# yex33/ReSpaSol

Measured on AMD Instinct MI355X. Metric: CSR SpMV GFLOP/s + achieved HBM GB/s (fp64 vs fp32), SuiteSparse set, 1/2/4/8 GPU, higher is better.
Workload: dtype f64; 1 GPU; big-set CSR SpMV fp64, 15 matrices per step; matrices=15, nnz_stored_total=268386865, parallelism=1 GPU, launch=rsp_spmv_batch (1 launch(es) of <= 32 matrices per step part): whole step

## Files before the change

### respasol_amd/csrc/rsp_api.cpp

```cpp

#include "rsp_internal.h"
#include "spmv_pack.h"

#include <atomic>

using namespace rsp_api;

using rsp::SpmvBlock;
using rsp::SpmvLongRow;
using rsp::SpmvTile;

namespace {
std::atomic<unsigned long long> g_plan_next{1};
unsigned long long plan_new_gen() { return g_plan_next.fetch_add(1); }
}


struct SpmvBounds {
    size_t nblocks, nlong, nslots;
};

static SpmvBounds spmv_bounds(int64_t rows, int64_t nnz, int cap) {
    SpmvBounds b;
    size_t q = (size_t)(nnz / cap) + 1;
    size_t l = (size_t)(nnz / rsp::kSpmvLongRow) + 1;
    b.nlong = q;
    b.nslots = 2 * q + 1;
    b.nblocks = 6 * q + 2 * l + (size_t)(rows / rsp::kSpmvMaxRows) + 8;
    b.nblocks += std::min<size_t>(b.nblocks, 8192);
    return b;
}

struct SpmvLayout {
    size_t off_long, off_part, off_cbase, off_poff, off_cidx, off_runs, bytes;
};
static SpmvLayout spmv_layout(const SpmvBounds &b, size_t elem, int64_t nnz, size_t run_ints = 0) {
    SpmvLayout l;
    l.off_long = align256(b.nblocks * sizeof(SpmvBlock));
    l.off_part = l.off_long + align256(b.nlong * sizeof(SpmvLongRow));
    l.off_cbase = l.off_part + align256(b.nslots * 2 * elem);
    l.off_poff = l.off_cbase + align256(b.nblocks * sizeof(int));
    l.off_cidx = l.off_poff + align256(b.nblocks * sizeof(int));
    l.off_runs = l.off_cidx + align256((size_t)std::max<int64_t>(nnz, 0) * sizeof(uint16_t));
    l.bytes = l.off_runs + align256(run_ints * sizeof(int));
    return l;
}

static int tile_cap(rsp_datatype_t t) {
    return t == RSP_R_64F ? SpmvTile<double>::kMaxNnz : SpmvTile<float>::kMaxNnz;
}
static int chunk_cap(rsp_datatype_t t) {
    return t == RSP_R_64F ? SpmvTile<double>::kChunk : SpmvTile<float>::kChunk;
}
static int spmv_row_align(rsp_handle_t h, rsp_datatype_t t) {
    const int e = (int)elem_size(t);
    return (h->spmv_variant & 64) ? 128 / e : (h->spmv_variant & 128) ? 64 / e : 1;
}

static int build_spmv_plan(const int *rp, int m, int cap, int chunk, rsp_an::hvec<SpmvBlock> &blocks,
                           rsp_an::hvec<SpmvLongRow> &longrows, int *nslots,
                           int maxrows = rsp::kSpmvMaxRows, int row_align = 1) {
    blocks.clear();
    longrows.clear();
    int slots = 0;
    int r = 0;
    while (r < m) {
        int len = rp[r + 1] - rp[r];
        if (len > rsp::kSpmvLongRow) {
            if (len <= chunk) {
                SpmvBlock b;
                b.r0 = r;
                b.r1 = rsp::kSpmvWholeRow;
                b.k0 = rp[r];
                b.k1 = rp[r + 1];
                blocks.push_back(b);
                r++;
                continue;
            }
            SpmvLongRow lr;
            lr.row = r;
            lr.first = slots;
            lr.nchunks = 0;
            lr.pad = 0;
            for (int k = rp[r]; k < rp[r + 1]; k += chunk) {
                SpmvBlock b;
                b.r0 = r;
                b.r1 = -(slots + 1);
                b.k0 = k;
                b.k1 = std::min(k + chunk, rp[r + 1]);
                blocks.push_back(b);
                slots++;
                lr.nchunks++;
            }
            longrows.push_back(lr);
            r++;
            continue;
        }
        int start = r, nnz = 0;
        while (r < m && r - start < maxrows) {
            int l = rp[r + 1] - rp[r];
            if (l > rsp::kSpmvLongRow || (r > start && nnz + l > cap)) break;
            nnz += l;
            r++;
        }
        if (row_align > 1 && r < m && r % row_align != 0) {
            const int ra = r - r % row_align;
            if (ra > start && (int64_t)(rp[ra] - rp[start]) * 4 >= (int64_t)(rp[r] - rp[start]) * 3) r = ra;
        }
        SpmvBlock b;
        b.r0 = start;
        b.r1 = r;
        b.k0 = rp[start];
        b.k1 = rp[r];
        blocks.push_back(b);
    }
    *nslots = slots;
    return 0;
}

struct TilePlan {
    rsp_an::hvec<SpmvBlock> blocks;
    rsp_an::hvec<SpmvLongRow> longrows;
    int nslots = 0, nint = 0;
    rsp_an::hvec<int> cbase;
    rsp_an::hvec<uint16_t> c16;
    rsp_an::hvec<int> runs;
    rsp_an::hvec<int> poff;
    int64_t nnz_c16 = 0;
    int64_t nnz_staged = 0;
    int64_t tiles_packed = 0, nnz_packed = 0;
};

static int spmv_pack_mode() { return std::min(std::max(env_int("RSP_SPMV_PACK", 2), 0), 2); }

template <typename T>
static void pack_staged_tiles(const int *rp, TilePlan &p, int mode) {
    constexpr int VW = SpmvTile<T>::kVec, IT = rsp::kSpmvIter, NTH = rsp::kSpmvThreads;
    constexpr int IW = rsp_pack::index_words(NTH, IT * VW);
    p.poff.assign(p.blocks.size(), -1);
    p.tiles_packed = p.nnz_packed = 0;
    if (mode <= 0) return;
    int64_t end = ((int64_t)p.runs.size() + 3) & ~(int64_t)3;
    for (size_t t = 0; t < p.blocks.size(); t++) {
        const SpmvBlock &b = p.blocks[t];
        if (p.cbase[t] > -2 || b.r1 < 0 || !rsp_pack::eligible(NTH, IT * VW, b.k1 - b.k0)) continue;
        const int64_t words = IW + (mode >= 2 ? rsp_pack::row_words(b.r1 - b.r0) : 0);
        if (end + words >= (1LL << 30)) break;
        p.poff[t] = (int)(end << 1) | (mode >= 2 ? 1 : 0);
        end = (end + words + 3) & ~(int64_t)3;
        p.tiles_packed++;
        p.nnz_packed += b.k1 - b.k0;
    }
    if (p.tiles_packed == 0) return;
    p.runs.resize((size_t)end + 4, 0);
    rsp_an::parallel_for((long long)p.blocks.size(), 64, [&](long long t0, long long t1) {
        for (long long t = t0; t < t1; t++) {
            if (p.poff[(size_t)t] < 0) continue;
            const SpmvBlock &b = p.blocks[(size_t)t];
            uint32_t *rec = reinterpret_cast<uint32_t *>(p.runs.data()) + (p.poff[(size_t)t] >> 1);
            rsp_pack::pack_slots(p.c16.data(), b.k0, b.k1, VW, IT, NTH, rec);
            if (p.poff[(size_t)t] & 1) rsp_pack::pack_rows(rp, b.r0, b.r1 - b.r0, b.k0 & ~(VW - 1), rec + IW);
        }
    });
}

static void make_tile_plan(const int *rp, const int *ci, int m, int64_t nnz_bound,
                           rsp_datatype_t type, int64_t spread, int64_t local_cols, bool use_c16,
                           TilePlan &p, int row_align = 1, bool use_stage = true) {
    const int chunk = chunk_cap(type);
    const int cap = tile_cap(type);
    const int align = row_align;
    const int maxrows = type == RSP_R_64F ? SpmvTile<double>::kMaxRows : SpmvTile<float>::kMaxRows;
    build_spmv_plan(rp, m, cap, chunk, p.blocks, p.longrows, &p.nslots, maxrows, align);
    const int64_t nb = (int64_t)p.blocks.size();
    if (spread > 0 && nb > 0 && nb < spread) {
        const SpmvBounds bb = spmv_bounds(m, std::max<int64_t>(nnz_bound, 0), chunk);
        const int64_t nnz_s = rp[(size_t)m];
        int c = (int)std::max<int64_t>(64, std::min<int64_t>(cap, (nnz_s + spread - 1) / spread));
        for (int tries = 0; tries < 32 && c < cap; tries++) {
            rsp_an::hvec<SpmvBlock> b2;
            rsp_an::hvec<SpmvLongRow> l2;
            int s2 = 0;
            build_spmv_plan(rp, m, c, chunk, b2, l2, &s2, maxrows, align);
            if ((int64_t)b2.size() <= spread && b2.size() <= bb.nblocks) {
                p.blocks.swap(b2);
                p.longrows.swap(l2);
                p.nslots = s2;
                break;
            }
            c += std::max(8, c / 16);
        }
    }
    const int ucap = type == RSP_R_64F ? SpmvTile<double>::kStageSlots : SpmvTile<float>::kStageSlots;
    const bool list_ok = use_stage && use_c16 && type == RSP_R_64F && SpmvTile<double>::kStageList &&
                         env_int("RSP_SPMV_STAGE_LIST", 1) != 0;
    if (list_ok && (int64_t)p.blocks.size() == nb && nb > 0) {
        int64_t band = 0, all = 0;
        std::vector<int> cols;
        const size_t step = std::max<size_t>(1, p.blocks.size() / 64);
        for (size_t t = 0; t < p.blocks.size(); t += step) {
            const SpmvBlock &bk = p.blocks[t];
            if (bk.r1 < 0 || bk.k1 <= bk.k0) continue;
            cols.assign(ci + bk.k0, ci + bk.k1);
            std::sort(cols.begin(), cols.end());
            cols.erase(std::unique(cols.begin(), cols.end()), cols.end());
            int R = 1;
            for (size_t u = 1; u < cols.size(); u++) R += cols[u] != cols[u - 1] + 1;
            all += bk.k1 - bk.k0;
            if (cols.back() - cols.front() <= 65535 && R > rsp::kStageRuns && (int)cols.size() > ucap)
                band += bk.k1 - bk.k0;
        }
        if (2 * band > all) {
            rsp_an::hvec<SpmvBlock> b2;
            rsp_an::hvec<SpmvLongRow> l2;
            int s2 = 0;
            const int lcap = std::min(std::max(env_int("RSP_SPMV_LIST_CAP", ucap), 64), ucap);
            build_spmv_plan(rp, m, std::min(cap, lcap), chunk, b2, l2, &s2, maxrows, align);
            p.blocks.swap(b2);
            p.longrows.swap(l2);
            p.nslots = s2;
        }
    }
    p.nint = 0;
    if (local_cols >= 0) {
        auto interior = [&](const SpmvBlock &b) {
            if (b.r1 < 0) return false;
            for (int k = b.k0; k < b.k1; k++)
                if (ci[(size_t)k] >= local_cols) return false;
            return true;
        };
        auto mid = std::stable_partition(p.blocks.begin(), p.blocks.end(), interior);
        p.nint = (int)(mid - p.blocks.begin());
    }
    const int64_t nnz_s = m > 0 ? rp[(size_t)m] : 0;
    p.cbase.assign(p.blocks.size(), -1);
    p.c16.clear();
    p.runs.clear();
    p.poff.assign(p.blocks.size(), -1);
    p.tiles_packed = p.nnz_packed = 0;
    p.nnz_c16 = 0;
    p.nnz_staged = 0;
    if (use_c16 && nnz_s > 0 && nnz_s <= nnz_bound) {
        p.c16.assign((size_t)nnz_s, 0);
        const long long nt = (long long)p.blocks.size();
        const long long pct = std::min(std::max(env_int("RSP_SPMV_STAGE_PCT", 80), 0), 100);
        const int64_t xelem = type == RSP_R_64F ? 8 : 4;
        std::vector<std::vector<int>> truns(use_stage ? (size_t)nt : 0);
        std::vector<char> tmode(use_stage ? (size_t)nt : 0, 0);
        std::atomic<int64_t> n16{0}, nst{0};
        rsp_an::parallel_for(nt, 64, [&](long long t0, long long t1) {
            std::vector<int> cols;
            int64_t c16n = 0, stn = 0;
            for (long long t = t0; t < t1; t++) {
                const SpmvBlock &bk = p.blocks[(size_t)t];
                if (bk.k1 <= bk.k0) continue;
                int lo = ci[(size_t)bk.k0], hi = lo;
                for (int k = bk.k0 + 1; k < bk.k1; k++) {
                    lo = std::min(lo, ci[(size_t)k]);
                    hi = std::max(hi, ci[(size_t)k]);
                }
                if (hi - lo > 65535) continue;
                const int len = bk.k1 - bk.k0;
                c16n += len;
                const bool x_in_rsrc = ((int64_t)hi + 1) * xelem <= (int64_t)0x7ffffffc;
                if (use_stage && bk.r1 >= 0 && x_in_rsrc) {
                    cols.assign(ci + bk.k0, ci + bk.k1);
                    std::sort(cols.begin(), cols.end());
                    cols.erase(std::unique(cols.begin(), cols.end()), cols.end());
                    const int U = (int)cols.size();
                    int R = 1;
                    for (int u = 1; u < U; u++) R += cols[(size_t)u] != cols[(size_t)u - 1] + 1;
                    const bool runs_mode = U <= ucap && R <= rsp::kStageRuns && 100LL * U <= pct * len;
                    const bool list_mode = !runs_mode && list_ok && U <= ucap && R > rsp::kStageRuns;
                    if (runs_mode || list_mode) {
                        std::vector<int> &r = truns[(size_t)t];
                        tmode[(size_t)t] = runs_mode ? 1 : 2;
                        if (runs_mode) {
                            r.reserve(2 * (size_t)(R + 1));
                            for (int u = 0; u < U; u++)
                                if (u == 0 || cols[(size_t)u] != cols[(size_t)u - 1] + 1) {
                                    r.push_back(cols[(size_t)u]);
                                    r.push_back(u);
                                }
                            r.push_back(0);
                            r.push_back(U);
                        } else {
                            r.assign(2 + 2 * (size_t)((U + 3) / 4), 0);
                            r[0] = cols[0];
                            r[1] = U;
                            uint16_t *o = reinterpret_cast<uint16_t *>(r.data() + 2);
                            for (int u = 0; u < U; u++) o[u] = (uint16_t)(cols[(size_t)u] - cols[0]);
                        }
                        for (int k = bk.k0; k < bk.k1; k++)
                            p.c16[(size_t)k] = (uint16_t)(std::lower_bound(cols.begin(), cols.end(), ci[(size_t)k]) -
                                                          cols.begin());
                        stn += len;
                        continue;
                    }
                }
                p.cbase[(size_t)t] = lo;
                for (int k = bk.k0; k < bk.k1; k++) p.c16[(size_t)k] = (uint16_t)(ci[(size_t)k] - lo);
            }
            n16 += c16n;
            nst += stn;
        });
        p.nnz_c16 = n16;
        p.nnz_staged = nst;
        if (use_stage) {
            for (size_t t = 0; t < truns.size(); t++) {
                const std::vector<int> &r = truns[t];
                if (r.empty()) continue;
                const int64_t off = (int64_t)p.runs.size() / 2;
                const int nr = tmode[t] == 2 ? 255 : (int)r.size() / 2 - 1;
                if (off >= (1LL << 22)) {
                    p.nnz_c16 -= p.blocks[t].k1 - p.blocks[t].k0;
                    p.nnz_staged -= p.blocks[t].k1 - p.blocks[t].k0;
                    continue;
                }
                p.cbase[t] = -2 - (int)((off << 8) | nr);
                p.runs.insert(p.runs.end(), r.begin(), r.end());
            }
            if (type == RSP_R_64F)
                pack_staged_tiles<double>(rp, p, spmv_pack_mode());
            else
                pack_staged_tiles<float>(rp, p, spmv_pack_mode());
        }
    }
}

static rsp_status_t download_pattern(rsp_handle_t h, rsp_spmat_t mat, rsp_an::hvec<int> &rp,
                                     rsp_an::hvec<int> &ci) {
    const int m = (int)mat->rows;
    rp.assign((size_t)m + 1, 0);
    ci.clear();
    if (m > 0) {
        RSP_CHECK_HIP(hipMemcpyAsync(rp.data(), mat->rowptr, ((size_t)m + 1) * sizeof(int),
                                     hipMemcpyDeviceToHost, h->stream));
        RSP_CHECK_HIP(hipStreamSynchronize(h->stream));
    }
    if (m > 0 && rp[0] != 0) return RSP_STATUS_INVALID_VALUE;
    for (int i = 0; i < m; i++)
        if (rp[i + 1] < rp[i]) return RSP_STATUS_INVALID_VALUE;
    if (m > 0 && (int64_t)rp[(size_t)m] > mat->nnz) return RSP_STATUS_INVALID_VALUE;
    if (m > 0 && rp[(size_t)m] > 0) {
        if (!mat->colidx) return RSP_STATUS_INVALID_VALUE;
        ci.resize((size_t)rp[(size_t)m]);
        RSP_CHECK_HIP(hipMemcpyAsync(ci.data(), mat->colidx, ci.size() * sizeof(int),
                                     hipMemcpyDeviceToHost, h->stream));
        RSP_CHECK_HIP(hipStreamSynchronize(h->stream));
        const int ncols = (int)mat->cols;
        for (int c : ci)
            if ((unsigned)c >= (unsigned)ncols) return RSP_STATUS_INVALID_VALUE;
    }
    return RSP_STATUS_SUCCESS;
}

static int64_t spmv_resident_tiles(rsp_handle_t h, rsp_datatype_t t) {
    return (int64_t)rsp_k::spmv_tiles_per_cu((int)elem_size(t)) * h->num_cus;
}

rsp_status_t rsp_api::spmv_plan(rsp_handle_t h, rsp_spmat_t mat, rsp_datatype_t compute_type) {
    const int m = (int)mat->rows;
    rsp_an::hvec<int> rp, ci;
    rsp_status_t st = download_pattern(h, mat, rp, ci);
    if (st != RSP_STATUS_SUCCESS) return st;
    const bool spread = (h->spmv_variant & 512) != 0;
    TilePlan p;
    make_tile_plan(rp.data(), ci.data(), m, mat->nnz, compute_type,
                   spread ? spmv_resident_tiles(h, compute_type) : 0,
                   mat->local_cols, !(h->spmv_variant & 32), p, spmv_row_align(h, compute_type),
                   !(h->spmv_variant & rsp::kSpmvVariantNoStage));
    const rsp_an::hvec<SpmvBlock> &blocks = p.blocks;
    const rsp_an::hvec<SpmvLongRow> &longrows = p.longrows;
    const int nslots = p.nslots, nint = p.nint;
    const rsp_an::hvec<int> &cbase = p.cbase;
    const rsp_an::hvec<uint16_t> &c16 = p.c16;
    const int64_t nnz_c16 = p.nnz_c16;
    SpmvBounds b{blocks.size(), longrows.size(), (size_t)nslots};
    const SpmvLayout lay = spmv_layout(b, elem_size(compute_type), (int64_t)c16.size(), p.runs.size());
    mat->planned = 0;
    if (lay.bytes > mat->plan_cap || !mat->d_plan) {
        if (mat->d_plan) {
            int cur = 0;
            (void)hipGetDevice(&cur);
            (void)hipSetDevice(mat->plan_device);
            (void)hipFree(mat->d_plan);
            (void)hipSetDevice(cur);
            mat->d_plan = nullptr;
            mat->plan_cap = 0;
        }
        RSP_CHECK_HIP(hipMalloc(&mat->d_plan, std::max<size_t>(lay.bytes, 256)));
        mat->plan_cap = std::max<size_t>(lay.bytes, 256);
        RSP_CHECK_HIP(hipGetDevice(&mat->plan_device));
    }
    char *buf = (char *)mat->d_plan;
    if (!blocks.empty()) {
        RSP_CHECK_HIP(hipMemcpyAsync(buf, blocks.data(), blocks.size() * sizeof(SpmvBlock),
                                     hipMemcpyHostToDevice, h->stream));
        RSP_CHECK_HIP(hipMemcpyAsync(buf + lay.off_cbase, cbase.data(), cbase.size() * sizeof(int),
                                     hipMemcpyHostToDevice, h->stream));
        RSP_CHECK_HIP(hipMemcpyAsync(buf + lay.off_poff, p.poff.data(), p.poff.size() * sizeof(int),
                                     hipMemcpyHostToDevice, h->stream));
    }
    if (!c16.empty())
        RSP_CHECK_HIP(hipMemcpyAsync(buf + lay.off_cidx, c16.data(), c16.size() * sizeof(uint16_t),
                                     hipMemcpyHostToDevice, h->stream));
    if (!p.runs.empty())
        RSP_CHECK_HIP(hipMemcpyAsync(buf + lay.off_runs, p.runs.data(), p.runs.size() * sizeof(int),
                                     hipMemcpyHostToDevice, h->stream));
    const size_t off_long = lay.off_long, off_part = lay.off_part;
    if (!longrows.empty())
        RSP_CHECK_HIP(hipMemcpyAsync(buf + off_long, longrows.data(),
                                     longrows.size() * sizeof(SpmvLongRow), hipMemcpyHostToDevice,
                                     h->stream));
    if (nslots > 0)
        RSP_CHECK_HIP(hipMemsetAsync(buf + off_part, 0, (size_t)nslots * 2 * elem_size(compute_type),
                                     h->stream));
    RSP_CHECK_HIP(hipStreamSynchronize(h->stream));
    mat->planned = 1;
    mat->plan_type = compute_type;
    mat->nblocks = (int)blocks.size();
    mat->nint = nint;
    mat->plan_gen = plan_new_gen();
    mat->nlong = (int)longrows.size();
    mat->nslots = nslots;
    mat->nnz_s = m > 0 ? rp[(size_t)m] : 0;
    mat->off_long = off_long;
    mat->off_part = off_part;
    mat->off_cbase = lay.off_cbase;
    mat->off_poff = lay.off_poff;
    mat->off_cidx = lay.off_cidx;
    mat->off_runs = lay.off_runs;
    mat->nnz_c16 = nnz_c16;
    mat->nnz_staged = p.nnz_staged;
    return RSP_STATUS_SUCCESS;
}

rsp_status_t rsp_api::spmv_run(rsp_handle_t h, rsp_operation_t op, const void *alpha, rsp_spmat_t mat,
                               const void *d_x, const void *beta, void *d_y,
                               rsp_datatype_t compute_type, void *d_buffer, int part) {
    if (!h) return RSP_STATUS_NOT_INITIALIZED;
    if (!mat || !alpha || !beta) return RSP_STATUS_INVALID_VALUE;
    if (op != RSP_OPERATION_NON_TRANSPOSE) return RSP_STATUS_NOT_SUPPORTED;
    if (compute_type != mat->type) return RSP_STATUS_INVALID_VALUE;
    if (mat->rows > 0 && (!d_y || (mat->cols > 0 && !d_x))) return RSP_STATUS_INVALID_VALUE;
    (void)d_buffer;
    if (!mat->planned || mat->plan_type != compute_type) {
        rsp_status_t st = spmv_plan(h, mat, compute_type);
        if (st != RSP_STATUS_SUCCESS) return st;
    }
    char *plan = (char *)mat->d_plan;
    rsp::SpmvArgs a;
    a.m = (int)mat->rows;
    a.rowptr = mat->rowptr;
    a.colidx = mat->colidx;
    a.vals = mat->vals;
    a.x = d_x;
    a.y = d_y;
    a.blocks = (const SpmvBlock *)plan;
    a.nblocks = mat->nblocks;
    a.cbases = (const int *)(plan + mat->off_cbase);
    a.poffs = (const int *)(plan + mat->off_poff);
    a.cidx = (const unsigned short *)(plan + mat->off_cidx);
    a.runs = (const int *)(plan + mat->off_runs);
    a.cmax = mat->cols > 0 ? (int)(mat->cols - 1) : 0;
    a.longrows = (const SpmvLongRow *)(plan + mat->off_long);
    a.nlong = mat->nlong;
    a.partials = plan + mat->off_part;
    if (compute_type == RSP_R_64F) {
        a.alpha = *(const double *)alpha;
        a.beta = *(const double *)beta;
    } else {
        a.alpha = *(const float *)alpha;
        a.beta = *(const float *)beta;
    }
    if (part != 0) {
        if (a.beta != 0.0) return RSP_STATUS_INVALID_VALUE;
        if (part == 1) {
            a.nblocks = mat->nint;
            a.nlong = 0;
        } else {
            a.blocks += mat->nint;
            a.cbases += mat->nint;
            a.poffs += mat->nint;
            a.nblocks = mat->nblocks - mat->nint;
        }
    }
    a.vector_ok = ((((uintptr_t)mat->colidx) | ((uintptr_t)mat->vals)) & 15) == 0;
    a.nnz = mat->nnz_s;
    a.variant = h->spmv_variant;
    hipError_t e;
    if (compute_type == RSP_R_64F)
        e = rsp_k::spmv_f64(a, h->stream);
    else
        e = h->ftz ? rsp_k_ftz::spmv_f32(a, h->stream) : rsp_k::spmv_f32(a, h->stream);
    return e == hipSuccess ? RSP_STATUS_SUCCESS : RSP_STATUS_EXECUTION_FAILED;
}


struct rsp_spmv_batch {
    rsp_datatype_t type;
    int part;
    rsp_an::hvec<rsp_spmat_t> mats;
    rsp_an::hvec<unsigned long long> plan_gen;
    rsp_an::hvec<rsp::SpmvBatchArgs> launches;
    void *d_mem = nullptr;
    int64_t tiles = 0, entries_16bit = 0;
    ~rsp_spmv_batch() {
        if (d_mem) (void)hipFree(d_mem);
    }
};

static rsp_status_t spmv_batch_create(rsp_handle_t h, int count, const rsp_spmat_t *mats,
                                      const void *const *d_x, void *const *d_y,
                                      void *const *d_buffers, rsp_datatype_t compute_type,
                                      int part, rsp_spmv_batch_t *batch) {
    if (!h) return RSP_STATUS_NOT_INITIALIZED;
    (void)d_buffers;
    if (!batch || count < 0 || (count > 0 && (!mats || !d_x || !d_y)))
        return RSP_STATUS_INVALID_VALUE;
    if (part < 0 || part > 2) return RSP_STATUS_INVALID_VALUE;
    if (compute_type != RSP_R_64F && compute_type != RSP_R_32F) return RSP_STATUS_INVALID_VALUE;
    *batch = nullptr;
    for (int j = 0; j < count; j++) {
        rsp_spmat_t A = mats[j];
        if (!A) return RSP_STATUS_INVALID_VALUE;
        if (A->type != compute_type) return RSP_STATUS_INVALID_VALUE;
        if (A->rows > 0 && (!d_y[j] || (A->cols > 0 && !d_x[j]))) return RSP_STATUS_INVALID_VALUE;
        if (!A->planned || A->plan_type != compute_type) {
            rsp_status_t st = spmv_plan(h, A, compute_type);
            if (st != RSP_STATUS_SUCCESS) return st;
        }
    }
    std::unique_ptr<rsp_spmv_batch> b(new rsp_spmv_batch());
    b->type = compute_type;
    b->part = part;
    const int64_t R = spmv_resident_tiles(h, compute_type);
    const bool spread_ok = !(h->spmv_variant & 16), c16_ok = !(h->spmv_variant & 32);
    const bool stage_ok = !(h->spmv_variant & rsp::kSpmvVariantNoStage);
    rsp_an::hvec<TilePlan> plans((size_t)count);
    struct Span { int first, count; size_t off_e, off_t, off_c, off_k, off_l; rsp_an::hvec<size_t> off_16, off_p, off_r; };
    rsp_an::hvec<Span> spans;
    size_t bytes = 0;
    auto tile_range = [part](const TilePlan &p, int *t0, int *t1) {
        *t0 = part == 2 ? p.nint : 0;
        *t1 = part == 1 ? p.nint : (int)p.blocks.size();
    };
    for (int first = 0; first < count; first += rsp::kSpmvBatchMax) {
        Span sp{first, std::min(rsp::kSpmvBatchMax, count - first), 0, 0, 0, 0, 0, {}, {}, {}};
        rsp_an::hvec<rsp_an::hvec<int>> rps((size_t)sp.count), cis((size_t)sp.count);
        int64_t nt_full = 0, nnz_all = 0;
        for (int q = 0; q < sp.count; q++) {
            rsp_spmat_t A = mats[first + q];
            rsp_status_t st = download_pattern(h, A, rps[q], cis[q]);
            if (st != RSP_STATUS_SUCCESS) return st;
            make_tile_plan(rps[q].data(), cis[q].data(), (int)A->rows, A->nnz, compute_type, 0,
                           A->local_cols, c16_ok, plans[first + q], spmv_row_align(h, compute_type), stage_ok);
            int t0, t1;
            tile_range(plans[first + q], &t0, &t1);
            nt_full += t1 - t0;
            nnz_all += A->rows > 0 ? rps[q][(size_t)A->rows] : 0;
        }
        if (spread_ok && nt_full < R)
            for (int q = 0; q < sp.count; q++) {
                rsp_spmat_t A = mats[first + q];
                const int64_t nnz_q = A->rows > 0 ? rps[q][(size_t)A->rows] : 0;
                const int64_t share = std::max<int64_t>(1, R * nnz_q / std::max<int64_t>(1, nnz_all));
                make_tile_plan(rps[q].data(), cis[q].data(), (int)A->rows, A->nnz, compute_type,
                               share, A->local_cols, c16_ok, plans[first + q],
                               spmv_row_align(h, compute_type), stage_ok);
            }
        int nt = 0, nl = 0;
        for (int q = 0; q < sp.count; q++) {
            const TilePlan &p = plans[first + q];
            rsp_spmat_t A = mats[first + q];
            if ((int)p.longrows.size() != A->nlong || p.nslots != A->nslots)
                return RSP_STATUS_INTERNAL_ERROR;
            int t0, t1;
            tile_range(p, &t0, &t1);
            nt += t1 - t0;
            nl += part == 1 ? 0 : (int)p.longrows.size();
        }
        sp.off_e = bytes;
        bytes += (size_t)sp.count * sizeof(rsp::SpmvBatchEntry);
        sp.off_t = bytes;
        bytes += (size_t)nt * sizeof(SpmvBlock);
        sp.off_c = bytes;
        bytes += ((size_t)nt * sizeof(int) + 15) & ~(size_t)15;
        sp.off_k = bytes;
        bytes += ((size_t)nt * sizeof(int) + 15) & ~(size_t)15;
        sp.off_l = bytes;
        bytes += ((size_t)nl * sizeof(SpmvLongRow) + 15) & ~(size_t)15;
        for (int q = 0; q < sp.count; q++) {
            sp.off_16.push_back(bytes);
            bytes += (plans[first + q].c16.size() * sizeof(uint16_t) + 15) & ~(size_t)15;
        }
        for (int q = 0; q < sp.count; q++) {
            sp.off_r.push_back(bytes);
            bytes += (plans[first + q].runs.size() * sizeof(int) + 15) & ~(size_t)15;
        }
        for (int q = 0; q < sp.count; q++) {
            sp.off_p.push_back(bytes);
            const size_t pb = (size_t)plans[first + q].nslots * 2 * elem_size(compute_type);
            bytes += (pb + 15) & ~(size_t)15;
        }
        spans.push_back(sp);
    }
    {
        size_t end = 0;
        auto region = [&](size_t off, size_t len) {
            const bool ok = off >= end && off + len <= bytes;
            end = off + len;
            return ok;
        };
        for (const Span &sp : spans) {
            int nt = 0, nl = 0;
            for (int q = 0; q < sp.count; q++) {
                int t0, t1;
                tile_range(plans[sp.first + q], &t0, &t1);
                nt += t1 - t0;
                nl += part == 1 ? 0 : (int)plans[sp.first + q].longrows.size();
            }
            bool ok = region(sp.off_e, (size_t)sp.count * sizeof(rsp::SpmvBatchEntry)) &&
                      region(sp.off_t, (size_t)nt * sizeof(SpmvBlock)) && region(sp.off_c, (size_t)nt * sizeof(int)) &&
                      region(sp.off_k, (size_t)nt * sizeof(int)) && region(sp.off_l, (size_t)nl * sizeof(SpmvLongRow));
            for (int q = 0; ok && q < sp.count; q++) ok = region(sp.off_16[q], plans[sp.first + q].c16.size() * 2);
            for (int q = 0; ok && q < sp.count; q++) ok = region(sp.off_r[q], plans[sp.first + q].runs.size() * 4);
            for (int q = 0; ok && q < sp.count; q++)
                ok = region(sp.off_p[q], (size_t)plans[sp.first + q].nslots * 2 * elem_size(compute_type));
            if (!ok) return RSP_STATUS_INTERNAL_ERROR;
        }
    }
    if (bytes > 0) RSP_CHECK_HIP(hipMalloc(&b->d_mem, bytes));
    rsp_an::hvec<unsigned char> host(bytes);
    for (const Span &sp : spans) {
        rsp::SpmvBatchArgs a{};
        a.entries = (const rsp::SpmvBatchEntry *)((char *)b->d_mem + sp.off_e);
        a.tiles = (const SpmvBlock *)((char *)b->d_mem + sp.off_t);
        a.cbases = (const int *)((char *)b->d_mem + sp.off_c);
        a.poffs = (const int *)((char *)b->d_mem + sp.off_k);
        a.longrows = (const SpmvLongRow *)((char *)b->d_mem + sp.off_l);
        a.count = sp.count;
        for (int q = 0; q <= rsp::kSpmvBatchMax; q++)
            a.tiles_at.begin[q] = a.longs_at.begin[q] = INT_MAX;
        int nt = 0, nl = 0;
        for (int q = 0; q < sp.count; q++) {
            rsp_spmat_t A = mats[sp.first + q];
            const TilePlan &p = plans[sp.first + q];
            int t0, t1;
            tile_range(p, &t0, &t1);
            const int nlq = part == 1 ? 0 : (int)p.longrows.size();
            rsp::SpmvBatchEntry e{};
            e.rowptr = A->rowptr;
            e.colidx = A->colidx;
            e.vals = A->vals;
            e.x = d_x[sp.first + q];
            e.y = d_y[sp.first + q];
            e.partials = (void *)((char *)b->d_mem + sp.off_p[q]);
            e.cidx = (const unsigned short *)((char *)b->d_mem + sp.off_16[q]);
            e.runs = (const int *)((char *)b->d_mem + sp.off_r[q]);
            e.cmax = A->cols > 0 ? (int)(A->cols - 1) : 0;
            e.nnz = A->nnz_s;
            e.vector_ok = ((((uintptr_t)A->colidx) | ((uintptr_t)A->vals)) & 15) == 0;
            memcpy(host.data() + sp.off_e + (size_t)q * sizeof(e), &e, sizeof(e));
            a.tiles_at.begin[q] = nt;
            a.longs_at.begin[q] = nl;
            for (int t = t0; t < t1; t++)
                if (p.cbase[(size_t)t] != -1) b->entries_16bit += p.blocks[(size_t)t].k1 - p.blocks[(size_t)t].k0;
            b->tiles += t1 - t0;
            if (t1 > t0) {
                memcpy(host.data() + sp.off_t + (size_t)nt * sizeof(SpmvBlock), p.blocks.data() + t0,
                       (size_t)(t1 - t0) * sizeof(SpmvBlock));
                memcpy(host.data() + sp.off_c + (size_t)nt * sizeof(int), p.cbase.data() + t0,
                       (size_t)(t1 - t0) * sizeof(int));
                memcpy(host.data() + sp.off_k + (size_t)nt * sizeof(int), p.poff.data() + t0,
                       (size_t)(t1 - t0) * sizeof(int));
            }
            if (nlq > 0)
                memcpy(host.data() + sp.off_l + (size_t)nl * sizeof(SpmvLongRow), p.longrows.data(),
                       (size_t)nlq * sizeof(SpmvLongRow));
            if (!p.c16.empty())
                memcpy(host.data() + sp.off_16[q], p.c16.data(), p.c16.size() * sizeof(uint16_t));
            if (!p.runs.empty())
                memcpy(host.data() + sp.off_r[q], p.runs.data(), p.runs.size() * sizeof(int));
            nt += t1 - t0;
            nl += nlq;
        }
        a.tiles_at.begin[sp.count] = nt;
        a.longs_at.begin[sp.count] = nl;
        b->launches.push_back(a);
    }
    if (bytes > 0) {
        RSP_CHECK_HIP(hipMemcpyAsync(b->d_mem, host.data(), bytes, hipMemcpyHostToDevice, h->stream));
        RSP_CHECK_HIP(hipStreamSynchronize(h->stream));
    }
    for (int j = 0; j < count; j++) {
        b->mats.push_back(mats[j]);
        b->plan_gen.push_back(mats[j]->plan_gen);
    }
    *batch = b.release();
    return RSP_STATUS_SUCCESS;
}

static void pack_geometry(rsp_datatype_t type, int *vw, int *iw) {
    *vw = type == RSP_R_64F ? SpmvTile<double>::kVec : SpmvTile<float>::kVec;
    *iw = rsp_pack::index_words(rsp::kSpmvThreads, rsp::kSpmvIter * *vw);
}

static rsp_status_t spmv_plan_stats(int m, const int *rp, const int *ci, int64_t nnz, rsp_datatype_t type,
                                    int64_t *out) {
    if (m < 0 || (m > 0 && (!rp || !ci)) || !out) return RSP_STATUS_INVALID_VALUE;
    if (type != RSP_R_64F && type != RSP_R_32F) return RSP_STATUS_NOT_SUPPORTED;
    TilePlan p;
    make_tile_plan(rp, ci, m, nnz, type, 0, -1, true, p);
    int vw, iw;
    pack_geometry(type, &vw, &iw);
    int64_t staged = 0, idx = 0, desc = 0, rows16 = 0, rowptr = 0;
    for (size_t t = 0; t < p.blocks.size(); t++) {
        const SpmvBlock &b = p.blocks[t];
        const int cb = p.cbase[t], po = p.poff[t];
        const int64_t len = b.k1 - b.k0, nrows = b.r1 > b.r0 ? b.r1 - b.r0 : 0;
        idx += po >= 0 ? 4LL * iw : cb == -1 ? 4 * len : 2 * len;
        if (cb <= -2) {
            const int code = -2 - cb, nr = code & 255;
            staged++;
            desc += nr == 255 ? 8 + 2LL * p.runs[2 * (size_t)(code >> 8) + 1] : 8LL * (nr + 1);
        }
        if (po >= 0 && (po & 1))
            rows16 += 4LL * rsp_pack::row_words((int)nrows);
        else
            rowptr += 4 * (nrows + 1);
    }
    out[0] = (int64_t)p.blocks.size();
    out[1] = p.tiles_packed;
    out[2] = p.nnz_packed;
    out[3] = 24 * (int64_t)p.blocks.size() + idx + desc + rows16;
    out[4] = rowptr;
    out[5] = staged;
    out[6] = idx;
    out[7] = rows16;
    return RSP_STATUS_SUCCESS;
}

static rsp_status_t spmv_plan_host(int m, const int *rp, const int *ci, int64_t nnz, rsp_datatype_t type,
                                   int64_t *tiles, int64_t *e16, int64_t *est) {
    if (m < 0 || (m > 0 && (!rp || !ci)) || !tiles || !e16 || !est) return RSP_STATUS_INVALID_VALUE;
    if (type != RSP_R_64F && type != RSP_R_32F) return RSP_STATUS_NOT_SUPPORTED;
    TilePlan p;
    make_tile_plan(rp, ci, m, nnz, type, 0, -1, true, p);
    const int ucap = type == RSP_R_64F ? SpmvTile<double>::kStageSlots : SpmvTile<float>::kStageSlots;
    int vw, iw;
    pack_geometry(type, &vw, &iw);
    const int pack_mode = spmv_pack_mode();
    if (p.poff.size() != p.blocks.size()) return RSP_STATUS_INTERNAL_ERROR;
    int64_t npk = 0, epk = 0;
    for (size_t t = 0; t < p.blocks.size(); t++) {
        const SpmvBlock &b = p.blocks[t];
        const int cb = p.cbase[t], po = p.poff[t];
        const uint32_t *rec = nullptr;
        if (po >= 0) {
            const int nrows = b.r1 - b.r0, kb = b.k0 & ~(vw - 1);
            const size_t w0 = (size_t)(po >> 1), words = (size_t)iw + ((po & 1) ? rsp_pack::row_words(nrows) : 0);
            if (cb > -2 || b.r1 < 0 || pack_mode == 0 || (po & 1) != (pack_mode >= 2) ||
                !rsp_pack::eligible(rsp::kSpmvThreads, rsp::kSpmvIter * vw, b.k1 - b.k0) || (w0 & 3) ||
                w0 + words > p.runs.size())
                return RSP_STATUS_INTERNAL_ERROR;
            rec = reinterpret_cast<const uint32_t *>(p.runs.data()) + w0;
            const int nwt = iw / rsp::kSpmvThreads;
            for (int tid = 0; tid < rsp::kSpmvThreads; tid++)
                for (int f = 0; f < rsp::kSpmvIter * vw; f++) {
                    const long long e = (long long)kb + (long long)((f / vw) * rsp::kSpmvThreads + tid) * vw + f % vw;
                    if ((e < b.k0 || e >= b.k1) && rsp_pack::get_field(rec + (size_t)tid * nwt, f) != 0)
                        return RSP_STATUS_INTERNAL_ERROR;
                }
            if (po & 1)
                for (int i = 0; i <= nrows; i++)
                    if (rsp_pack::unpack_row(rec + iw, i) + kb != rp[b.r0 + i]) return RSP_STATUS_INTERNAL_ERROR;
            npk++;
            epk += b.k1 - b.k0;
        }
        auto slot_of = [&](int k) {
            return rec ? (int)rsp_pack::unpack_slot(rec, b.k0, k, vw, rsp::kSpmvIter, rsp::kSpmvThreads)
                       : (int)p.c16[(size_t)k];
        };
        if (cb == -1) continue;
        for (int k = b.k0; k < b.k1; k++) {
            int col;
            if (cb >= 0) {
                col = cb + p.c16[(size_t)k];
            } else {
                const int code = -2 - cb, nr = code & 255, off = code >> 8;
                if (nr == 255) {
                    if (type != RSP_R_64F) return RSP_STATUS_INTERNAL_ERROR;
                    if ((size_t)2 * off + 2 > p.runs.size()) return RSP_STATUS_INTERNAL_ERROR;
                    const int *r = p.runs.data() + 2 * (size_t)off;
                    const int U = r[1];
                    if (U < 1 || U > ucap || (size_t)2 * off + 2 + 2 * (size_t)((U + 3) / 4) > p.runs.size())
                        return RSP_STATUS_INTERNAL_ERROR;
                    const uint16_t *o = reinterpret_cast<const uint16_t *>(r + 2);
                    for (int u = 1; u < U; u++)
                        if (o[u] <= o[u - 1]) return RSP_STATUS_INTERNAL_ERROR;
                    const int u = slot_of(k);
                    if (u >= U) return RSP_STATUS_INTERNAL_ERROR;
                    if (r[0] + o[u] != ci[k]) return RSP_STATUS_INTERNAL_ERROR;
                    continue;
                }
                if (nr < 1 || nr > rsp::kStageRuns || (size_t)2 * (off + nr + 1) > p.runs.size())
                    return RSP_STATUS_INTERNAL_ERROR;
                const int *r = p.runs.data() + 2 * (size_t)off;
                const int U = r[2 * nr + 1];
                if (r[1] != 0 || U > ucap) return RSP_STATUS_INTERNAL_ERROR;
                for (int j = 1; j <= nr; j++)
                    if (r[2 * j + 1] <= r[2 * j - 1] || (j < nr && r[2 * j] <= r[2 * j - 2] + (r[2 * j + 1] - r[2 * j - 1]) - 1))
                        return RSP_STATUS_INTERNAL_ERROR;
                const int u = slot_of(k);
                if (u >= U) return RSP_STATUS_INTERNAL_ERROR;
                int j = 0;
                while (j + 1 < nr && r[2 * (j + 1) + 1] <= u) j++;
                col = r[2 * j] + (u - r[2 * j + 1]);
            }
            if (col != ci[k]) return RSP_STATUS_INTERNAL_ERROR;
        }
    }
    if (npk != p.tiles_packed || epk != p.nnz_packed) return RSP_STATUS_INTERNAL_ERROR;
    *tiles = (int64_t)p.blocks.size();
    *e16 = p.nnz_c16;
    *est = p.nnz_staged;
    return RSP_STATUS_SUCCESS;
}

extern "C" {

int rsp_get_version(void) { return RSP_VERSION_MAJOR * 1000 + RSP_VERSION_MINOR; }

const char *rsp_get_error_string(rsp_status_t s) {
    switch (s) {
        case RSP_STATUS_SUCCESS: return "RSP_STATUS_SUCCESS";
        case RSP_STATUS_NOT_INITIALIZED: return "RSP_STATUS_NOT_INITIALIZED";
        case RSP_STATUS_ALLOC_FAILED: return "RSP_STATUS_ALLOC_FAILED";
        case RSP_STATUS_INVALID_VALUE: return "RSP_STATUS_INVALID_VALUE";
        case RSP_STATUS_ARCH_MISMATCH: return "RSP_STATUS_ARCH_MISMATCH";
        case RSP_STATUS_EXECUTION_FAILED: return "RSP_STATUS_EXECUTION_FAILED";
        case RSP_STATUS_INTERNAL_ERROR: return "RSP_STATUS_INTERNAL_ERROR";
        case RSP_STATUS_MATRIX_TYPE_NOT_SUPPORTED: return "RSP_STATUS_MATRIX_TYPE_NOT_SUPPORTED";
        case RSP_STATUS_ZERO_PIVOT: return "RSP_STATUS_ZERO_PIVOT";
        case RSP_STATUS_NOT_SUPPORTED: return "RSP_STATUS_NOT_SUPPORTED";
    }
    return "RSP_STATUS_UNKNOWN";
}

rsp_status_t rsp_create(rsp_handle_t *handle) {
    if (!handle) return RSP_STATUS_INVALID_VALUE;
    *handle = nullptr;
    int dev = 0;
    if (hipGetDevice(&dev) != hipSuccess) return RSP_STATUS_NOT_INITIALIZED;
    hipDeviceProp_t prop;
    if (hipGetDeviceProperties(&prop, dev) != hipSuccess) return RSP_STATUS_NOT_INITIALIZED;
    if (strncmp(prop.gcnArchName, "gfx950", 6) != 0) return RSP_STATUS_ARCH_MISMATCH;
    rsp_context *c = new (std::nothrow) rsp_context;
    if (!c) return RSP_STATUS_ALLOC_FAILED;
    c->device = dev;
    c->stream = nullptr;
    c->ftz = 0;
    const char *v = getenv("RSP_SPMV_VARIANT");
    c->spmv_variant = v ? atoi(v) : 0;
    c->num_cus = prop.multiProcessorCount > 0 ? prop.multiProcessorCount : 256;
    rsp_k::warm_spmv();
    rsp_k_ftz::warm_spmv();
    rsp_k::warm_ilu();
    rsp_k_ftz::warm_ilu();
    rsp_k::warm_analysis();
    rsp_k::warm_krylov();
    rsp_k_ftz::warm_krylov();
    c->d_ftrace = nullptr;
    c->d_strace = nullptr;
    c->d_dot = nullptr;
    c->h_dot = nullptr;
    c->d_gm = nullptr;
    c->h_gm = nullptr;
    *handle = c;
    return RSP_STATUS_SUCCESS;
}

rsp_status_t rsp_destroy(rsp_handle_t h) {
    if (!h) return RSP_STATUS_NOT_INITIALIZED;
    if (h->d_ftrace || h->d_strace || h->d_dot || h->h_dot || h->d_gm || h->h_gm) {
        int cur = 0;
        (void)hipGetDevice(&cur);
        (void)hipSetDevice(h->device);
        if (h->d_ftrace) (void)hipFree(h->d_ftrace);
        if (h->d_strace) (void)hipFree(h->d_strace);
        if (h->d_dot) (void)hipFree(h->d_dot);
        if (h->h_dot) (void)hipHostFree(h->h_dot);
        if (h->d_gm) (void)hipFree(h->d_gm);
        if (h->h_gm) (void)hipHostFree(h->h_gm);
        (void)hipSetDevice(cur);
    }
    delete h;
    return RSP_STATUS_SUCCESS;
}

rsp_status_t rsp_set_stream(rsp_handle_t h, void *stream) {
    if (!h) return RSP_STATUS_NOT_INITIALIZED;
    h->stream = (hipStream_t)stream;
    return RSP_STATUS_SUCCESS;
}

rsp_status_t rsp_get_stream(rsp_handle_t h, void **stream) {
    if (!h) return RSP_STATUS_NOT_INITIALIZED;
    if (!stream) return RSP_STATUS_INVALID_VALUE;
    *stream = (void *)h->stream;
    return RSP_STATUS_SUCCESS;
}

rsp_status_t rsp_set_ftz(rsp_handle_t h, int enable) {
    if (!h) return RSP_STATUS_NOT_INITIALIZED;
    h->ftz = enable ? 1 : 0;
    return RSP_STATUS_SUCCESS;
}

rsp_status_t rsp_get_ftz(rsp_handle_t h, int *enable) {
    if (!h) return RSP_STATUS_NOT_INITIALIZED;
    if (!enable) return RSP_STATUS_INVALID_VALUE;
    *enable = h->ftz;
    return RSP_STATUS_SUCCESS;
}


rsp_status_t rsp_create_csr(rsp_spmat_t *mat, int64_t rows, int64_t cols, int64_t nnz,
                            void *d_row_offsets, void *d_col_ind, void *d_values,
                            rsp_datatype_t value_type) {
    if (!mat) return RSP_STATUS_INVALID_VALUE;
    *mat = nullptr;
    if (rows < 0 || cols < 0 || nnz < 0 || rows > INT_MAX - 1 || cols > INT_MAX || nnz > INT_MAX)
        return RSP_STATUS_INVALID_VALUE;
    if (value_type != RSP_R_64F && value_type != RSP_R_32F) return RSP_STATUS_INVALID_VALUE;
    if (!d_row_offsets && rows > 0) return RSP_STATUS_INVALID_VALUE;
    if ((!d_col_ind || !d_values) && nnz > 0) return RSP_STATUS_INVALID_VALUE;
    rsp_spmat *a = new (std::nothrow) rsp_spmat;
    if (!a) return RSP_STATUS_ALLOC_FAILED;
    memset(a, 0, sizeof(*a));
    a->rows = rows;
    a->cols = cols;
    a->nnz = nnz;
    a->rowptr = (int *)d_row_offsets;
    a->colidx = (int *)d_col_ind;
    a->vals = d_values;
    a->type = value_type;
    a->planned = 0;
    a->d_plan = nullptr;
    a->local_cols = -1;
    *mat = a;
    return RSP_STATUS_SUCCESS;
}

rsp_status_t rsp_spmat_set_local_cols(rsp_spmat_t mat, int64_t ncols_local) {
    if (!mat || ncols_local < 0 || ncols_local > mat->cols) return RSP_STATUS_INVALID_VALUE;
    mat->local_cols = ncols_local;
    mat->planned = 0;
    return RSP_STATUS_SUCCESS;
}

rsp_status_t rsp_csr_set_values(rsp_spmat_t mat, void *d_values, rsp_datatype_t value_type) {
    if (!mat) return RSP_STATUS_INVALID_VALUE;
    if (value_type != RSP_R_64F && value_type != RSP_R_32F) return RSP_STATUS_INVALID_VALUE;
    if (d_values != mat->vals) mat->plan_gen = plan_new_gen();
    mat->vals = d_values;
    if (value_type != mat->type) mat->planned = 0;
    mat->type = value_type;
    return RSP_STATUS_SUCCESS;
}

rsp_status_t rsp_destroy_spmat(rsp_spmat_t mat) {
    if (!mat) return RSP_STATUS_INVALID_VALUE;
    if (mat->d_plan) {
        int cur = 0;
        (void)hipGetDevice(&cur);
        (void)hipSetDevice(mat->plan_device);
        (void)hipFree(mat->d_plan);
        (void)hipSetDevice(cur);
    }
    delete mat;
    return RSP_STATUS_SUCCESS;
}


rsp_status_t rsp_spmv_buffer_size(rsp_handle_t h, rsp_operation_t op, const void *alpha,
                                  rsp_spmat_t mat, const void *beta, rsp_datatype_t compute_type,
                                  size_t *buffer_size) {
    (void)alpha;
    (void)beta;
    return guarded([&] {
        if (!h) return RSP_STATUS_NOT_INITIALIZED;
        if (!mat || !buffer_size) return RSP_STATUS_INVALID_VALUE;
        if (op != RSP_OPERATION_NON_TRANSPOSE) return RSP_STATUS_NOT_SUPPORTED;
        if (compute_type != mat->type) return RSP_STATUS_INVALID_VALUE;
        if (!mat->planned || mat->plan_type != compute_type) RSP_TRY(spmv_plan(h, mat, compute_type));
        *buffer_size = 0;
        return RSP_STATUS_SUCCESS;
    });
}

rsp_status_t rsp_spmv_preprocess(rsp_handle_t h, rsp_operation_t op, const void *alpha,
                                 rsp_spmat_t mat, const void *d_x, const void *beta, void *d_y,
                                 rsp_datatype_t compute_type, void *d_buffer) {
    (void)alpha;
    (void)beta;
    (void)d_x;
    (void)d_y;
    (void)d_buffer;
    return guarded([&] {
        if (!h) return RSP_STATUS_NOT_INITIALIZED;
        if (!mat) return RSP_STATUS_INVALID_VALUE;
        if (op != RSP_OPERATION_NON_TRANSPOSE) return RSP_STATUS_NOT_SUPPORTED;
        if (compute_type != mat->type) return RSP_STATUS_INVALID_VALUE;
        return spmv_plan(h, mat, compute_type);
    });
}

rsp_status_t rsp_spmv_plan_info(rsp_spmat_t mat, int64_t *tiles, int64_t *entries_16bit) {
    if (!mat || !tiles || !entries_16bit) return RSP_STATUS_INVALID_VALUE;
    if (!mat->planned) return RSP_STATUS_NOT_INITIALIZED;
    *tiles = mat->nblocks;
    *entries_16bit = mat->nnz_c16;
    return RSP_STATUS_SUCCESS;
}

rsp_status_t rsp_spmv(rsp_handle_t h, rsp_operation_t op, const void *alpha, rsp_spmat_t mat,
                      const void *d_x, const void *beta, void *d_y, rsp_datatype_t compute_type,
                      void *d_buffer) {
    return guarded([&] { return spmv_run(h, op, alpha, mat, d_x, beta, d_y, compute_type, d_buffer, 0); });
}

rsp_status_t rsp_spmv_part(rsp_handle_t h, const void *alpha, rsp_spmat_t mat, const void *d_x,
                           const void *beta, void *d_y, rsp_datatype_t compute_type,
                           void *d_buffer, int part) {
    return guarded([&] {
        if (part < 0 || part > 2) return RSP_STATUS_INVALID_VALUE;
        return spmv_run(h, RSP_OPERATION_NON_TRANSPOSE, alpha, mat, d_x, beta, d_y, compute_type,
                        d_buffer, part);
    });
}


rsp_status_t rsp_spmv_batch_create(rsp_handle_t h, int count, const rsp_spmat_t *mats,
                                   const void *const *d_x, void *const *d_y,
                                   void *const *d_buffers, rsp_datatype_t compute_type,
                                   int part, rsp_spmv_batch_t *batch) {
    return guarded([&] { return spmv_batch_create(h, count, mats, d_x, d_y, d_buffers, compute_type, part, batch); });
}

rsp_status_t rsp_spmv_batch_run(rsp_handle_t h, rsp_spmv_batch_t b, const void *alpha,
                                const void *beta) {
    if (!h) return RSP_STATUS_NOT_INITIALIZED;
    if (!b || !alpha || !beta) return RSP_STATUS_INVALID_VALUE;
    for (size_t j = 0; j < b->mats.size(); j++) {
        const rsp_spmat_t A = b->mats[j];
        if (!A->planned || A->plan_gen != b->plan_gen[j]) return RSP_STATUS_INVALID_VALUE;
    }
    const double av = b->type == RSP_R_64F ? *(const double *)alpha : *(const float *)alpha;
    const double bv = b->type == RSP_R_64F ? *(const double *)beta : *(const float *)beta;
    if (b->part != 0 && bv != 0.0) return RSP_STATUS_INVALID_VALUE;
    for (rsp::SpmvBatchArgs a : b->launches) {
        a.alpha = av;
        a.beta = bv;
        a.variant = h->spmv_variant;
        hipError_t e;
        if (b->type == RSP_R_64F)
            e = rsp_k::spmv_batch_f64(a, h->stream);
        else
            e = h->ftz ? rsp_k_ftz::spmv_batch_f32(a, h->stream) : rsp_k::spmv_batch_f32(a, h->stream);
        if (e != hipSuccess) return RSP_STATUS_EXECUTION_FAILED;
    }
    return RSP_STATUS_SUCCESS;
}

rsp_status_t rsp_spmv_batch_info(rsp_spmv_batch_t b, int64_t *tiles, int64_t *entries_16bit) {
    if (!b || !tiles || !entries_16bit) return RSP_STATUS_INVALID_VALUE;
    *tiles = b->tiles;
    *entries_16bit = b->entries_16bit;
    return RSP_STATUS_SUCCESS;
}

rsp_status_t rsp_spmv_batch_destroy(rsp_spmv_batch_t b) {
    if (!b) return RSP_STATUS_INVALID_VALUE;
    delete b;
    return RSP_STATUS_SUCCESS;
}

rsp_status_t rsp_gather(rsp_handle_t h, rsp_datatype_t value_type, int64_t n, const int64_t *d_idx,
                        const void *d_src, void *d_dst) {
    if (!h) return RSP_STATUS_NOT_INITIALIZED;
    if (value_type != RSP_R_64F && value_type != RSP_R_32F) return RSP_STATUS_INVALID_VALUE;
    if (n < 0 || (n > 0 && (!d_idx || !d_src || !d_dst))) return RSP_STATUS_INVALID_VALUE;
    hipError_t e = rsp_k::gather(value_type == RSP_R_64F ? 8 : 4, n, d_idx, d_src, d_dst, h->stream);
    return e == hipSuccess ? RSP_STATUS_SUCCESS : RSP_STATUS_EXECUTION_FAILED;
}

rsp_status_t rsp_scatter(rsp_handle_t h, rsp_datatype_t value_type, int64_t n, const int64_t *d_idx,
                         const void *d_src, void *d_dst) {
    if (!h) return RSP_STATUS_NOT_INITIALIZED;
    if (value_type != RSP_R_64F && value_type != RSP_R_32F) return RSP_STATUS_INVALID_VALUE;
    if (n < 0 || (n > 0 && (!d_idx || !d_src || !d_dst))) return RSP_STATUS_INVALID_VALUE;
    hipError_t e = rsp_k::scatter(value_type == RSP_R_64F ? 8 : 4, n, d_idx, d_src, d_dst, h->stream);
    return e == hipSuccess ? RSP_STATUS_SUCCESS : RSP_STATUS_EXECUTION_FAILED;
}

rsp_status_t rsp_spmv_plan_host(int m, const int *row_offsets, const int *col_ind, int64_t nnz,
                                rsp_datatype_t compute_type, int64_t *tiles, int64_t *entries_16bit,
                                int64_t *entries_staged) {
    return guarded([&] {
        return spmv_plan_host(m, row_offsets, col_ind, nnz, compute_type, tiles, entries_16bit, entries_staged);
    });
}

rsp_status_t rsp_spmv_plan_stats(int m, const int *row_offsets, const int *col_ind, int64_t nnz,
                                 rsp_datatype_t compute_type, int64_t stats[8]) {
    return guarded([&] { return spmv_plan_stats(m, row_offsets, col_ind, nnz, compute_type, stats); });
}

}
```

### respasol_amd/csrc/rsp_internal.h

```cpp
#pragma once

#include "rsp.h"

#include <hip/hip_runtime.h>
#include <limits.h>
#include <math.h>
#include <stdio.h>
#include <stdlib.h>
#include <string.h>

#include <algorithm>
#include <cmath>
#include <memory>
#include <new>
#include <vector>

#include "rsp_kernels.h"
#include "ilu_analysis.h"

struct rsp_context {
    int device;
    hipStream_t stream;
    int ftz;
    int spmv_variant;
    int num_cus;
    unsigned long long *d_ftrace;
    unsigned long long *d_strace;
    double *d_dot;
    double *h_dot;
    double *d_gm;
    double *h_gm;
};

struct rsp_spmat {
    int64_t rows, cols, nnz;
    int *rowptr;
    int *colidx;
    void *vals;
    rsp_datatype_t type;
    int planned;
    int plan_device;
    void *d_plan;
    size_t plan_cap;
    rsp_datatype_t plan_type;
    int nblocks, nlong, nslots;
    int nnz_s;
    size_t off_long, off_part;
    size_t off_cbase, off_poff, off_cidx, off_runs;
    int64_t nnz_c16;
    int64_t nnz_staged;
    int64_t local_cols;
    int nint;
    unsigned long long plan_gen;
};

struct rsp_ilu0_info {
    int analysed;
    int n, nnz_s;
    const int *rowptr, *colidx;
    int structural_zero;
    int factored;
    int *d_dpos, *d_hasdiag;
    int *d_upd_ptr, *d_upd_l, *d_upd_u, *d_lord, *d_lend, *d_udiv;
    int *d_zero;
    unsigned long long claim_host = 0;
    int *d_fdone = nullptr;
    unsigned *d_tk = nullptr;
    unsigned long long tk_seq = 0;
    unsigned flow_epoch = 0;
    int solve_gen[3] = {0, 0, 0};
    long long n_updates;
    struct Dag {
        rsp_an::hvec<int> ptr;
        int *d_rows = nullptr, *d_ptr = nullptr;
        rsp::RowTask *d_tasks = nullptr;
        int *d_tpos = nullptr, *d_src = nullptr;
        rsp::LevelChunk *d_chunks = nullptr;
        rsp::ThinRowPlan *d_trow = nullptr;
        int *d_sid = nullptr;
        rsp::StagedTerm *d_stg = nullptr;
        rsp::FlowItem *d_fitems = nullptr;
        int nterms = 0;
        int *d_nshort = nullptr;
        rsp_an::hvec<int> nshort;
        rsp_an::hvec<int> nwave;
        rsp_an::hvec<int> sbase;
        rsp_an::hvec<rsp::LevelSeg> segs;
        int batch = 8;
        int group = 4;
    } L, LT, U, F;
    struct BlkDag {
        bool on = false;
        int nb = 0, lds_elems = 0, lds_words = 0, entries = 0, nlong = 0;
        rsp_an::hvec<rsp::BlkSeg> segs;
        int *d_order = nullptr, *d_ref = nullptr, *d_vpos = nullptr, *d_lptr = nullptr, *d_rptr = nullptr;
        rsp::BlkDesc *d_desc = nullptr;
        rsp::BlkRow *d_rows = nullptr;
        unsigned *d_eord = nullptr, *d_rit = nullptr;
        void *d_ev = nullptr, *d_yp = nullptr;
        void *d_rc = nullptr;
    } Lb, LTb;
    bool fac_one = false, fac_scale = false;
    const Dag &fdag() const { return fac_one ? F : L; }
    rsp_an::hvec<rsp::LevelSeg> fac_segs;
    void *d_sval = nullptr, *d_sx = nullptr, *d_sdg = nullptr;
    rsp::RndChunk *d_rchunks = nullptr;
    rsp::RndItem *d_ritems = nullptr;
    rsp::FacRow *d_frow = nullptr;
    int *d_fslots = nullptr;
    rsp_an::hvec<rsp::FacFlowRun> fruns;
    rsp::FacFlowItem *d_ffitems = nullptr;
    void *d_forig = nullptr;
    int fac_gen = 0;
    rsp_an::hvec<rsp::FacSlotLevel> fslev;
    int *d_rpairs = nullptr, *d_rstaged = nullptr, *d_rrounds = nullptr;
    int fac_batch;
    void *d_arena = nullptr;
    void *d_arena_u = nullptr;
    void *d_arena_sym = nullptr;
    void *d_arena_pairs = nullptr;
    void *d_usval = nullptr;
    unsigned long long digest = 0;
    std::unique_ptr<rsp_an::IluHostPlan> host;
    rsp_an::hvec<int> host_rp, host_ci;
    std::unique_ptr<rsp_an::Task> solves_task;
    bool solves_ready = false;
    bool dev_terms = true;
    void *d_arena_s = nullptr;
    rsp_handle_t han = nullptr;
    void *d_fbackup = nullptr;
    size_t fbackup_bytes = 0;
    long long call_seq = 0;
    struct FacCall {
        long long seq = 0;
        int valid = 0;
        int ftz = 0;
        rsp_datatype_t type = RSP_R_64F;
        void *vals = nullptr;
    } last_fac;
    struct SolveCall {
        long long seq = 0;
        int valid = 0;
        int ftz = 0;
        rsp_operation_t op = RSP_OPERATION_NON_TRANSPOSE;
        double alpha = 1.0;
        rsp_datatype_t type = RSP_R_64F;
        const void *vals = nullptr, *x = nullptr;
        void *y = nullptr;
    } last_solve[3];
};

#define RSP_CHECK_HIP(call)                                                     \
    do {                                                                        \
        hipError_t e_ = (call);                                                 \
        if (e_ != hipSuccess)                                                   \
            return e_ == hipErrorOutOfMemory ? RSP_STATUS_ALLOC_FAILED          \
                                             : RSP_STATUS_EXECUTION_FAILED;     \
    } while (0)

#define RSP_TRY(call)                                   \
    do {                                                \
        const rsp_status_t st_ = (call);                \
        if (st_ != RSP_STATUS_SUCCESS) return st_;      \
    } while (0)

namespace rsp_api {

using rsp_an::env_int;

template <typename F, typename C>
rsp_status_t guarded(F body, C cleanup) {
    try {
        return body();
    } catch (const std::bad_alloc &) {
        cleanup();
        return RSP_STATUS_ALLOC_FAILED;
    } catch (...) {
        cleanup();
        return RSP_STATUS_INTERNAL_ERROR;
    }
}
template <typename F>
rsp_status_t guarded(F body) {
    return guarded(body, [] {});
}

inline size_t align256(size_t x) { return (x + 255) & ~(size_t)255; }
inline size_t elem_size(rsp_datatype_t t) { return t == RSP_R_64F ? 8 : 4; }

rsp_status_t spmv_plan(rsp_handle_t h, rsp_spmat_t mat, rsp_datatype_t compute_type);
rsp_status_t spmv_run(rsp_handle_t h, rsp_operation_t op, const void *alpha, rsp_spmat_t mat, const void *d_x,
                      const void *beta, void *d_y, rsp_datatype_t compute_type, void *d_buffer, int part);

rsp_status_t ilu_solves_ready(rsp_handle_t h, rsp_ilu0_info *f);
rsp_status_t ilu_plan_u(rsp_handle_t h, rsp_ilu0_info *f);

rsp_status_t rsp_trsv_lower_unit_impl(rsp_handle_t h, rsp_operation_t op, const void *alpha, rsp_ilu0_info_t f,
                                      rsp_datatype_t value_type, const void *d_values, const void *d_x, void *d_y,
                                      bool flow_ok);
rsp_status_t rsp_trsv_upper_impl(rsp_handle_t h, const void *alpha, rsp_ilu0_info_t f, rsp_datatype_t value_type,
                                 const void *d_values, const void *d_x, void *d_y, bool flow_ok);

}
```

### respasol_amd/csrc/rsp_kernels.h

```cpp
#pragma once

#include <hip/hip_runtime.h>
#include <stdint.h>

namespace rsp {

struct alignas(16) SpmvBlock {
    int r0, r1, k0, k1;
};

struct alignas(16) SpmvLongRow {
    int row, first, nchunks, pad;
};

#ifndef RSP_SPMV_THREADS
#define RSP_SPMV_THREADS 256
#endif
constexpr int kSpmvThreads = RSP_SPMV_THREADS;
#ifndef RSP_SPMV_ITER
#define RSP_SPMV_ITER 4
#endif
constexpr int kSpmvIter = RSP_SPMV_ITER;
#ifndef RSP_SPMV_MAXROWS
#define RSP_SPMV_MAXROWS 512
#endif
constexpr int kSpmvMaxRows = RSP_SPMV_MAXROWS;
constexpr int kSpmvLongRow = 256;
constexpr int kSpmvHeavyMax = 128;
constexpr int kSpmvWholeRow = -2147483647 - 1;
template <typename T>
struct SpmvTile {
    static constexpr int kVec = 16 / sizeof(T);
    static constexpr int kSlots = kSpmvThreads * kSpmvIter * kVec;
    static constexpr int kMaxNnz = kSlots - (kVec - 1);
    static constexpr int kChunk = kSpmvThreads * 4 * kVec - (kVec - 1);
    static_assert(kChunk <= kMaxNnz, "a chunk must fit one tile");
    static constexpr int kMaxRows = sizeof(T) == 8 ? kSpmvMaxRows : 2 * kSpmvMaxRows;
    static constexpr int kStageSlots = sizeof(T) == 8 ? 1536 : 2048;
    static constexpr bool kStageList = sizeof(T) == 8;
};
static_assert(SpmvTile<float>::kMaxNnz / 33 < kSpmvHeavyMax && SpmvTile<double>::kMaxNnz / 33 < kSpmvHeavyMax,
              "every > 32-entry row of a tile fits the heavy-row list");
constexpr int kStageRuns = 254;

struct SpmvArgs {
    int m;
    const int *rowptr;
    const int *colidx;
    const void *vals;
    const void *x;
    void *y;
    const SpmvBlock *blocks;
    int nblocks;
    const int *cbases;
    const unsigned short *cidx;
    const int *runs;
    const int *poffs;
    int cmax;
    const SpmvLongRow *longrows;
    int nlong;
    void *partials;
    double alpha, beta;
    int nnz;
    int vector_ok;
    int variant;
};

constexpr int kSpmvBatchMax = 32;
struct alignas(16) SpmvBatchEntry {
    const int *rowptr;
    const int *colidx;
    const void *vals;
    const void *x;
    void *y;
    void *partials;
    const unsigned short *cidx;
    const int *runs;
    int nnz;
    int vector_ok;
    int cmax;
};
struct SpmvBatchTable {
    int begin[kSpmvBatchMax + 1];
};
struct SpmvBatchArgs {
    const SpmvBatchEntry *entries;
    const SpmvBlock *tiles;
    const int *cbases;
    const int *poffs;
    const SpmvLongRow *longrows;
    int count;
    SpmvBatchTable tiles_at, longs_at;
    double alpha, beta;
    int variant;
};
constexpr int kSpmvVariantFixup = 256;
constexpr int kSpmvVariantNoStage = 1024;

struct LevelSeg {
    int lb, le, thin, c0, c1;
    int nth;
};
struct alignas(16) RowTask {
    int i, t0, t1, d;
};
struct alignas(16) LevelChunk {
    int l0, l1;
    int x0, x1;
    int k0, k1;
    int st0, st1;
};
struct alignas(16) FlowItem {
    int x0, n, t0, gate;
};
struct alignas(16) ThinRowPlan {
    int g, out, i, d;
};
struct alignas(8) StagedTerm {
    int slot, j;
};

struct LevelPlan {
    const int *rows;
    const int *ptr_dev;
    const int *ptr_host;
    int nlev;
    const LevelSeg *segs;
    int nseg;
    int batch;
    int group;
    const RowTask *tasks;
    const int *tpos;
    const int *src;
    const LevelChunk *chunks;
    const ThinRowPlan *trow;
    const int *sid;
    const StagedTerm *stg;
    const FlowItem *fitems;
    int has_flow;
    int nterms;
    const int *nshort;
    const int *nshort_host;
    const int *nwave_host;
    const int *sbase_host;
};
constexpr int kLongTerms = 64;
constexpr int kHubTerms = 256;
constexpr int kFatLongTerms = 8;
constexpr int kFatLongDefault = 3;
constexpr int kYWin = 4096;
constexpr int kChunkRows = 1024;
constexpr int kChunkTerms = 4096;
constexpr int kThinThreads = 1024;
constexpr int kGroup = 4;
constexpr int kPadSrc = -(kYWin + 1);
constexpr int kIluWaves = 4;
constexpr int kFacRow = 256;
constexpr int kFacPairs = 1024;
constexpr int kThinSolveRows = 512;
constexpr int kThinSolveTerms = 2048;
constexpr int kThinFactorRows = 1024;
constexpr int kRndItems = 2048;
constexpr int kRndPairs = 4096;
constexpr int kRndStaged = 4096;
constexpr int kRndRounds = 2048;
constexpr int kRndLevelItems = 1 << 15;
constexpr int kRndFlowItems = 1024;
constexpr int kRndItemPairs = 1024;
constexpr int kRndLevelStart = 1 << 15;
struct alignas(16) RndChunk {
    int i0, i1, p0, p1, s0, s1, r0, r1;
};
struct alignas(16) RndItem {
    int pos, u, d, zr;
};

struct alignas(16) FacRow {
    int i, rs, di, re, q0, q1, hasdiag, pad;
};

struct FacSlotLevel {
    long long off;
    int stride, rm, qm, pad;
};
__host__ __device__ constexpr int fac_pairs_at(int rm) { return (8 + 2 * rm + 1) & ~1; }

struct alignas(16) FacFlowItem {
    long long off;
    int rmqm, gate;
};
struct FacFlowRun {
    int lb, le, c0, c1;
};

struct FlowCtl {
    int *status;
    int gen;
    unsigned long long ticks;
    unsigned long long *claim;
    unsigned long long *claim_host;
    int mode;
    unsigned *tickets;
    unsigned long long *tk_seq;
    int *done;
    int grid_x;
    unsigned epoch;
};
constexpr int kFlowClaims = 1;
constexpr int kFlowTickets = 2;
constexpr int kFlowTicketCtrs = 8;
constexpr int kFlowOwnMax = 1024;
#ifndef RSP_TK_STEAL_US
#define RSP_TK_STEAL_US 50
#endif
constexpr int kFlowStealUs = RSP_TK_STEAL_US;


struct IluArgs {
    int n;
    const int *rowptr;
    const int *colidx;
    const int *dpos;
    const int *hasdiag;
    void *vals;
    int *zero_pivot;
    const int *upd_ptr;
    const int *upd_l;
    const int *upd_u;
    const int *lord;
    const int *lend;
    const int *udiv;
    const FacRow *frow;
    const int *fslots;
    const FacSlotLevel *fslev;
    int fat_slots;
    int fat_lds;
    LevelPlan plan;
    const RndChunk *rchunks;
    const RndItem *ritems;
    const int *rpairs, *rstaged, *rrounds;
    unsigned long long *trace;
    int trace_cap;
    int defer_rounds;
    int narrow_waves;
    const FacFlowItem *fitems;
    const FacFlowRun *fruns;
    int nfruns;
    const int *lev;
    void *forig;
    int gen;
    int flow, flow_grid, flow_sleep;
    int flow_cus;
    FlowCtl fc;
    int fac_one;
};

constexpr int kBlkRows = 64, kBlkYMax = 32, kBlkNear = 12, kBlkNearWin = 1 << 30, kBlkWin = 16384;
constexpr int kBlkLongCap = 64 * kBlkNear;
constexpr int kBlkPre = 6;
struct alignas(16) BlkDesc {
    int p0, np, kind, kn;
    int eoff, ne, doff, nd;
    int loff, nlev, ovf, pad;
};
struct alignas(16) BlkRow {
    int off, nx, ny, nfar;
};
struct BlkSeg {
    int b0, b1, p0, p1;
};
struct BlkArgs {
    int n, nb;
    const int *order;
    const BlkDesc *desc;
    const BlkRow *rows;
    const int *ref;
    const int *vpos;
    const unsigned *eord;
    const int *lptr;
    const int *rptr;
    const unsigned *rit;
    const BlkSeg *segs;
    int nseg;
    int lds_elems;
    int lds_words;
    const void *vals, *x;
    void *y;
    double alpha;
    void *ev, *yp;
    void *rc;
};

struct TrsvArgs {
    int n;
    const int *rowptr;
    const int *colidx;
    const int *dpos;
    const int *hasdiag;
    const void *vals;
    const void *x;
    void *y;
    double alpha;
    LevelPlan plan;
    void *sval;
    void *sx;
    void *sdg;
    unsigned long long *trace;
    int trace_cap;
    int trace_clk;
    int wave_lds;
    int narrow_waves;
    int narrow_split;
    int narrow_pairs;
    int loaders;
    int flow;
    int flow_grid;
    int flow_cus;
    FlowCtl fc;
    int flow_sleep;
};


constexpr int kKryThreads = 256;
constexpr int kKryChunk = 2048;
constexpr int kKryMaxGrid = 1024;
struct KryGrid {
    int grid;
    long long chunk;
};
inline KryGrid kry_grid(long long n) {
    KryGrid g;
    const long long span = (long long)kKryChunk * kKryMaxGrid;
    g.chunk = (long long)kKryChunk * (n > span ? (n + span - 1) / span : 1);
    g.grid = n > 0 ? (int)((n + g.chunk - 1) / g.chunk) : 1;
    return g;
}
enum {
    kKryRho0 = 0,
    kKryRho1 = 1,
    kKryAlpha = 2,
    kKryOmega = 3,
    kKryFlag = 4,
    kKryFlagIt = 5,
    kKryScalars = 16
};
enum { kKryPartRR = 0, kKryPartBB, kKryPartRhR, kKryPartRhV, kKryPartTS, kKryPartTT, kKryDots };
enum { kKryBreakRho = 1, kKryBreakOmega = 2, kKryBreakRhV = 3, kKryBreakTT = 4 };
constexpr size_t kKryBlockDoubles = kKryScalars + (size_t)kKryDots * kKryMaxGrid;
enum KryOp {
    kKryInit,
    kKryPUpdate,
    kKryDotRhV,
    kKrySUpdate,
    kKryDotTS,
    kKryXUpdate,
    kKryWiden,
    kKryZero,
    kKryDot
};
enum { kKryF64 = 0, kKryF32 = 1, kKryF64Copy32 = 2 };
struct KryArgs {
    long long n;
    double *blk;
    int it;
    const void *b;
    const void *c;
    void *x, *r, *rhat, *p, *v, *s, *t;
    const void *phat, *shat;
    void *copy32;
};
inline double kry_combine_host(const double *part, int g) {
    double v[kKryThreads];
    for (int t = 0; t < kKryThreads; t++) {
        v[t] = 0.0;
        for (int i = t; i < g; i += kKryThreads) v[t] += part[i];
    }
    double w[kKryThreads / 64];
    for (int k = 0; k < kKryThreads / 64; k++) {
        double *l = v + 64 * k;
        for (int off = 32; off > 0; off >>= 1)
            for (int i = 0; i < off; i++) l[i] += l[i + off];
        w[k] = l[0];
    }
    return ((w[0] + w[1]) + w[2]) + w[3];
}

constexpr int kGmMax = 64;
constexpr int kGmLd = kGmMax + 1;
enum {
    kGmStop = 0,
    kGmDone = 1,
    kGmBeta = 2,
    kGmBn = 3,
    kGmFlag = kKryFlag,
    kGmFlagIt = kKryFlagIt,
    kGmScalars = 16,
    kGmEst = kGmScalars,
    kGmHead = kGmEst + kGmMax,
    kGmR = kGmHead,
    kGmCs = kGmR + kGmLd * kGmMax,
    kGmSn = kGmCs + kGmMax,
    kGmG = kGmSn + kGmMax,
    kGmY = kGmG + kGmLd,
    kGmH1 = kGmY + kGmMax,
    kGmH2 = kGmH1 + kGmLd,
    kGmSmall = (kGmH2 + kGmLd + 15) / 16 * 16
};
enum {
    kGmPartRR = 0,
    kGmPartBB = 1,
    kGmPartNrm = 2,
    kGmPartD1 = 3,
    kGmPartD2 = kGmPartD1 + kGmLd,
    kGmDots = kGmPartD2 + kGmLd
};
enum { kGmBreakH = 1, kGmBreakDiag = 2, kGmBreakNorm = 3, kGmBreakY = 4 };
constexpr size_t kGmBlockDoubles = kGmSmall + (size_t)kGmDots * kKryMaxGrid;
enum GmOp {
    kGmResid,
    kGmNormalise,
    kGmMultiDot,
    kGmUpdate1,
    kGmUpdate2,
    kGmCombine
};
struct GmArgs {
    long long n;
    double *blk;
    int j;
    int first;
    const void *b;
    void *x;
    void *V;
    long long ldv;
    const void *Z;
    long long ldz;
    void *w;
    void *copy32;
};

#if defined(__HIPCC__)
#define RSP_HD __host__ __device__
#else
#define RSP_HD
#endif
RSP_HD inline int gmres_lsq(double *col, int j, double *cs, double *sn, double *g, const double *R, int ldr,
                            int k, double *y) {
    if (col) {
        for (int i = 0; i <= j + 1; i++)
            if (!(col[i] - col[i] == 0.0)) return kGmBreakH;
        for (int i = 0; i < j; i++) {
            const double a = col[i], b = col[i + 1];
            col[i] = cs[i] * a + sn[i] * b;
            col[i + 1] = cs[i] * b - sn[i] * a;
        }
        const double a = col[j], b = col[j + 1];
        const double aa = a < 0.0 ? -a : a, ab = b < 0.0 ? -b : b;
        const double s = aa > ab ? aa : ab;
        if (s == 0.0) return kGmBreakDiag;
        const double as = a / s, bs = b / s;
        const double r = s * sqrt(as * as + bs * bs);
        if (r == 0.0 || !(r - r == 0.0)) return kGmBreakDiag;
        const double c = a / r, t = b / r;
        cs[j] = c;
        sn[j] = t;
        col[j] = r;
        col[j + 1] = 0.0;
        const double gj = g[j];
        g[j] = c * gj;
        g[j + 1] = -(t * gj);
    }
    if (y) {
        for (int i = k - 1; i >= 0; i--) {
            double v = g[i];
            for (int l = i + 1; l < k; l++) v -= R[i + (size_t)l * ldr] * y[l];
            y[i] = v / R[i + (size_t)i * ldr];
        }
    }
    return 0;
}
}

#define RSP_DECLARE_KERNEL_API(NS)                                                              \
    namespace NS {                                                                              \
    hipError_t spmv_f32(const rsp::SpmvArgs &a, hipStream_t s);                                 \
    hipError_t spmv_batch_f32(const rsp::SpmvBatchArgs &a, hipStream_t s);                      \
    hipError_t ilu0_factor_f32(const rsp::IluArgs &a, hipStream_t s);                           \
    hipError_t trsv_lower_n_f32(const rsp::TrsvArgs &a, hipStream_t s);                         \
    hipError_t trsv_lower_t_f32(const rsp::TrsvArgs &a, hipStream_t s);                         \
    hipError_t trsv_upper_f32(const rsp::TrsvArgs &a, hipStream_t s);                           \
    hipError_t trsv_blocks_f32(const rsp::BlkArgs &a, hipStream_t s);                           \
    void warm_spmv();                                                                           \
    void warm_ilu();                                                                            \
    hipError_t krylov(rsp::KryOp op, int type, const rsp::KryArgs &a, hipStream_t s);           \
    hipError_t gmres(rsp::GmOp op, int type, const rsp::GmArgs &a, hipStream_t s);              \
    void warm_krylov();                                                                         \
    }

RSP_DECLARE_KERNEL_API(rsp_k)
RSP_DECLARE_KERNEL_API(rsp_k_ftz)

namespace rsp_k {
hipError_t gather(int elem_bytes, int64_t n, const int64_t *idx, const void *src, void *dst,
                  hipStream_t s);
hipError_t scatter(int elem_bytes, int64_t n, const int64_t *idx, const void *src, void *dst,
                   hipStream_t s);
hipError_t spmv_f64(const rsp::SpmvArgs &a, hipStream_t s);
hipError_t spmv_batch_f64(const rsp::SpmvBatchArgs &a, hipStream_t s);
int spmv_tiles_per_cu(int elem_bytes);
void warm_analysis();
hipError_t ilu0_factor_f64(const rsp::IluArgs &a, hipStream_t s);
hipError_t trsv_lower_n_f64(const rsp::TrsvArgs &a, hipStream_t s);
hipError_t trsv_lower_t_f64(const rsp::TrsvArgs &a, hipStream_t s);
hipError_t trsv_upper_f64(const rsp::TrsvArgs &a, hipStream_t s);
hipError_t trsv_blocks_f64(const rsp::BlkArgs &a, hipStream_t s);
hipError_t ilu0_build_slots(const rsp::IluArgs &a, const int4 *desc, const long long *offs, int nrows,
                            int *slots, hipStream_t s);
hipError_t ilu_an_rows(int n, const int *rp, const int *ci, int *dpos, int *hasdiag, int *flags, hipStream_t s);
hipError_t ilu_an_count(const int *const rows_c[3], const int n_c[3], int cap0, const int *rp, const int *ci,
                        const int *dpos, const int *hasdiag, int *cnt, int *gcur, hipStream_t s);
hipError_t ilu_an_scan(const int *cnt, int *ptr, int count, void *temp, size_t *temp_bytes, hipStream_t s);
hipError_t ilu_an_gather_pairs(const int *rows, int nrows, const int *rp, const int *ptr, const int *cbase,
                               const int *upd_l, const int *upd_u, int *out_l, int *out_u, hipStream_t s);
hipError_t ilu_an_fill(const int *const rows_c[3], const int n_c[3], int cap0, const int *rp, const int *ci,
                       const int *dpos, const int *hasdiag, const int *ptr, int *gcur, int *upd_l, int *upd_u,
                       hipStream_t s);
hipError_t ilu_an_stages(int n, int maxlen, const int *rp, const int *ci, const int *dpos, const int *hasdiag,
                         const int *ptr, const int *upd_l, int *stage, int *lord, int *lend, int *udiv,
                         int *scratch, const int *wrows, int nwrows, hipStream_t s);
struct SolveTermsArgs {
    int kind, n, nx, total, nch, group;
    const rsp::RowTask *tasks;
    const int *ptr;
    const int *rp, *ci, *dpos;
    const int *ltp, *lts, *ltc;
    const int *lpos;
    const int *ne;
    rsp::LevelChunk *chunks;
    const int *cbase;
    int *tpos, *src, *sid;
    rsp::ThinRowPlan *trow;
    rsp::StagedTerm *stg;
    int *slot_of, *nst, *nst_ptr;
    void *scan;
};
hipError_t ilu_an_solve_terms(const SolveTermsArgs &a, hipStream_t s);
}
```

### respasol_amd/csrc/spmv.hip

```cpp

#include <hip/hip_runtime.h>

#include <type_traits>

#include "rsp_kernels.h"
#include "spmv_pack.h"

#ifndef RSP_KNS
#define RSP_KNS rsp_k
#endif

#ifndef RSP_NT_Y
#define RSP_NT_Y -1
#endif

namespace RSP_KNS {

using rsp::kSpmvThreads;
using rsp::kSpmvHeavyMax;
using rsp::SpmvArgs;
using rsp::SpmvBlock;
using rsp::SpmvLongRow;
using rsp::SpmvTile;
using rsp::kSpmvBatchMax;
using rsp::SpmvBatchArgs;
using rsp::SpmvBatchEntry;
using rsp::SpmvBatchTable;

template <typename T, int N>
struct VecT;
template <>
struct VecT<double, 2> {
    typedef double __attribute__((ext_vector_type(2))) V;
    typedef int __attribute__((ext_vector_type(2))) I;
    typedef unsigned short __attribute__((ext_vector_type(2))) H;
};
template <>
struct VecT<float, 4> {
    typedef float __attribute__((ext_vector_type(4))) V;
    typedef int __attribute__((ext_vector_type(4))) I;
    typedef unsigned short __attribute__((ext_vector_type(4))) H;
};

__device__ __forceinline__ int xcd_swizzle(int bid, int nwg) {
    const int q = nwg >> 3, r = nwg & 7;
    const int xcd = bid & 7, idx = bid >> 3;
    const int start = xcd < r ? xcd * (q + 1) : r * (q + 1) + (xcd - r) * q;
    return start + idx;
}

template <bool NT, typename P>
__device__ __forceinline__ P ld(const P *p) {
    if constexpr (NT)
        return __builtin_nontemporal_load(p);
    else
        return *p;
}

template <typename T, bool NT, bool C16 = false, int NTH = kSpmvThreads,
          int IT = SpmvTile<T>::kSlots / (kSpmvThreads * (16 / sizeof(T)))>
__device__ __forceinline__ void stream_products(const int *__restrict__ colidx,
                                                const unsigned short *__restrict__ cidx, int cbase,
                                                int cmax, const T *__restrict__ vals,
                                                const T *__restrict__ x, int kb, int k1,
                                                T *__restrict__ lds) {
    constexpr int VW = 16 / sizeof(T);
    typedef typename VecT<T, VW>::V V;
    typedef typename VecT<T, VW>::I I;
    typedef typename VecT<T, VW>::H H;
    const int tid = threadIdx.x;
    const int last = (k1 - 1) & ~(VW - 1);
    I ci[IT];
    H ch[IT];
#pragma unroll
    for (int it = 0; it < IT; ++it) {
        const int e = min(kb + (it * NTH + tid) * VW, last);
        if constexpr (C16)
            ch[it] = ld<NT>(reinterpret_cast<const H *>(cidx + e));
        else
            ci[it] = ld<NT>(reinterpret_cast<const I *>(colidx + e));
    }
    V vv[IT];
#pragma unroll
    for (int it = 0; it < IT; ++it) {
        const int e = min(kb + (it * NTH + tid) * VW, last);
        vv[it] = ld<NT>(reinterpret_cast<const V *>(vals + e));
    }
    __builtin_amdgcn_sched_barrier(0);
    T xv[IT][VW];
#pragma unroll
    for (int it = 0; it < IT; ++it)
#pragma unroll
        for (int j = 0; j < VW; ++j) {
            int c;
            if constexpr (C16)
                c = min(cbase + (int)ch[it][j], cmax);
            else
                c = ci[it][j];
            xv[it][j] = x[c];
        }
    __builtin_amdgcn_sched_barrier(0);
#pragma unroll
    for (int it = 0; it < IT; ++it) {
        V p;
#pragma unroll
        for (int j = 0; j < VW; ++j) p[j] = vv[it][j] * xv[it][j];
        *reinterpret_cast<V *>(lds + (it * NTH + tid) * VW) = p;
    }
}

__device__ __forceinline__ void lds_barrier() {
    __builtin_amdgcn_fence(__ATOMIC_RELEASE, "workgroup", "local");
    __builtin_amdgcn_s_barrier();
    __builtin_amdgcn_fence(__ATOMIC_ACQUIRE, "workgroup", "local");
}

template <typename T, bool NT, int PKM, int NTH = kSpmvThreads,
          int IT = SpmvTile<T>::kSlots / (kSpmvThreads * (16 / sizeof(T)))>
__device__ __forceinline__ void stream_products_staged(const unsigned short *__restrict__ cidx,
                                                       const unsigned int *__restrict__ pk, int2 rd,
                                                       int nr, const int (&lsl)[SpmvTile<T>::kStageSlots / NTH],
                                                       const T *__restrict__ vals,
                                                       const T *__restrict__ x, int kb, int k1,
                                                       T *__restrict__ lds) {
    constexpr int VW = 16 / sizeof(T);
    constexpr int SMAX = SpmvTile<T>::kStageSlots / NTH;
    typedef typename VecT<T, VW>::V V;
    const int tid = threadIdx.x;
    const int last = (k1 - 1) & ~(VW - 1);
    constexpr int NW = rsp_pack::words_per_thread(IT * VW);
    constexpr int HW = VW / 2;
    static_assert(NW <= IT * HW, "the packed words fit the unpacked ones' registers");
    const bool pkd = PKM == 2 ? pk != nullptr : PKM == 1;
    unsigned int iw[PKM == 1 ? NW : IT * HW];
    V vv[IT];
    if (pkd) {
        const unsigned int *w = pk + tid * NW;
#pragma unroll
        for (int q = 0; q < NW; ++q) iw[q] = ld<NT>(w + q);
    } else {
#pragma unroll
        for (int it = 0; it < IT; ++it) {
            const int e = min(kb + (it * NTH + tid) * VW, last);
            const unsigned int *w = reinterpret_cast<const unsigned int *>(cidx + e);
#pragma unroll
            for (int q = 0; q < HW; ++q) iw[it * HW + q] = ld<NT>(w + q);
        }
    }
#pragma unroll
    for (int it = 0; it < IT; ++it) {
        const int e = min(kb + (it * NTH + tid) * VW, last);
        vv[it] = ld<NT>(reinterpret_cast<const V *>(vals + e));
    }
    __builtin_amdgcn_sched_barrier(0);
    const __amdgpu_buffer_rsrc_t xr =
        __builtin_amdgcn_make_buffer_rsrc((void *)x, (short)0, 0x7ffffffc, 0x00020000);
    auto xload = [&](int col) {
        if constexpr (sizeof(T) == 8)
            return __builtin_bit_cast(T, __builtin_amdgcn_raw_buffer_load_b64(xr, col * 8, 0, 0));
        else
            return __builtin_bit_cast(T, __builtin_amdgcn_raw_buffer_load_b32(xr, col * 4, 0, 0));
    };
    T xs[SMAX];
    int U;
    if (SpmvTile<T>::kStageList && nr == 255) {
        U = rd.y;
#pragma unroll
        for (int k = 0; k < SMAX; ++k)
            if (k * NTH < U) xs[k] = xload(rd.x + lsl[k]);
    } else {
        int2 *tab = reinterpret_cast<int2 *>(lds + SpmvTile<T>::kSlots) - (nr + 1);
        if (tid <= nr) tab[tid] = rd;
        lds_barrier();
        U = tab[nr].y;
        int us[SMAX], lo[SMAX];
#pragma unroll
        for (int k = 0; k < SMAX; ++k) {
            us[k] = min(k * NTH + tid, U - 1);
            lo[k] = 0;
        }
        for (int n = nr; n > 1;) {
            const int h = n >> 1;
#pragma unroll
            for (int k = 0; k < SMAX; ++k)
                if (tab[lo[k] + h].y <= us[k]) lo[k] += h;
            n -= h;
        }
#pragma unroll
        for (int k = 0; k < SMAX; ++k)
            if (k * NTH < U) {
                const int2 r = tab[lo[k]];
                xs[k] = xload(r.x + (us[k] - r.y));
            }
    }
#pragma unroll
    for (int k = 0; k < SMAX; ++k)
        if (k * NTH < U && k * NTH + tid < U) lds[k * NTH + tid] = xs[k];
    lds_barrier();
    T xv[IT][VW];
    if (pkd) {
#pragma unroll
        for (int it = 0; it < IT; ++it)
#pragma unroll
            for (int j = 0; j < VW; ++j) xv[it][j] = lds[min((int)rsp_pack::get_field(iw, it * VW + j), U - 1)];
    } else {
#pragma unroll
        for (int it = 0; it < IT; ++it)
#pragma unroll
            for (int j = 0; j < VW; ++j)
                xv[it][j] = lds[min((int)((iw[(it * VW + j) >> 1] >> (16 * (j & 1))) & 0xffffu), U - 1)];
    }
    lds_barrier();
#pragma unroll
    for (int it = 0; it < IT; ++it) {
        V p;
#pragma unroll
        for (int j = 0; j < VW; ++j) p[j] = vv[it][j] * xv[it][j];
        *reinterpret_cast<V *>(lds + (it * NTH + tid) * VW) = p;
    }
}

template <typename T, int NTH = kSpmvThreads>
__device__ __forceinline__ void stream_products_scalar(const int *__restrict__ colidx,
                                                       const T *__restrict__ vals,
                                                       const T *__restrict__ x, int k0, int kb,
                                                       int k1, T *lds) {
    for (int e = kb + (int)threadIdx.x; e < k1; e += NTH)
        if (e >= k0) lds[e - kb] = vals[e] * x[colidx[e]];
}

template <typename T, int L, int NTH, typename Sink>
__device__ __forceinline__ void reduce_rows(const T *lds, const unsigned short *rp_lds, int nrows, int kb,
                                            int heavy, int *hl, int *hn, Sink sink) {
    constexpr int NA = 8 / L;
    constexpr int NG = NTH / L;
    const int tid = threadIdx.x;
    const int g = tid / L, lane = tid & (L - 1);
    for (int rr = g; rr - g < nrows; rr += NG) {
        bool active = rr < nrows;
        T acc[NA];
#pragma unroll
        for (int t = 0; t < NA; ++t) acc[t] = T(0);
        if (active) {
            const int a0 = rp_lds[rr] - kb, a1 = rp_lds[rr + 1] - kb, last = a1 - 1;
            if (heavy > 0 && a1 - a0 > heavy) {
                active = false;
                if (lane == 0) hl[atomicAdd(hn, 1)] = rr;
            } else {
                for (int base = a0 + lane; base < a1; base += 8) {
                    T v[NA];
#pragma unroll
                    for (int t = 0; t < NA; ++t) v[t] = lds[min(base + t * L, last)];
#pragma unroll
                    for (int t = 0; t < NA; ++t)
                        acc[t] = base + t * L < a1 ? acc[t] + v[t] : acc[t];
                }
            }
        }
#pragma unroll
        for (int h = NA / 2; h >= 1; h >>= 1)
#pragma unroll
            for (int t = 0; t < h; ++t) acc[t] = acc[t] + acc[t + h];
        T s = acc[0];
#pragma unroll
        for (int off = L / 2; off >= 1; off >>= 1) s = s + __shfl_xor(s, off, 64);
        if (active && lane == 0) sink(rr, s);
    }
}

template <typename T, int NTH, typename Sink>
__device__ __forceinline__ void reduce_heavy_rows(const T *lds, const unsigned short *rp_lds, int kb,
                                                  const int *hl, int hn, Sink sink) {
    constexpr int NG = NTH / 8;
    const int tid = threadIdx.x;
    const int g = tid >> 3, lane = tid & 7;
    for (int h = g; h - g < hn; h += NG) {
        const bool active = h < hn;
        T acc = T(0);
        const int rr = active ? hl[h] : 0;
        if (active) {
            const int a1 = rp_lds[rr + 1] - kb, last = a1 - 1;
            for (int base = rp_lds[rr] - kb + lane; base < a1; base += 32) {
                T v[4];
#pragma unroll
                for (int t = 0; t < 4; ++t) v[t] = lds[min(base + 8 * t, last)];
#pragma unroll
                for (int t = 0; t < 4; ++t) acc = base + 8 * t < a1 ? acc + v[t] : acc;
            }
        }
#pragma unroll
        for (int off = 4; off >= 1; off >>= 1) acc = acc + __shfl_xor(acc, off, 64);
        if (active && lane == 0) sink(rr, acc);
    }
}

template <typename T, int NTH = kSpmvThreads, typename Sink>
__device__ __forceinline__ void reduce_tile_rows(const T *lds, const unsigned short *rp_lds, int nrows,
                                                 int nnzt, int kb, int *hl, int *hn, Sink sink) {
    int L = 1;
    while (L < 8 && 2 * L * nrows <= NTH && 8 * L * nrows <= nnzt) L <<= 1;
    switch (L) {
        case 1: reduce_rows<T, 1, NTH>(lds, rp_lds, nrows, kb, 32, hl, hn, sink); break;
        case 2: reduce_rows<T, 2, NTH>(lds, rp_lds, nrows, kb, 64, hl, hn, sink); break;
        case 4: reduce_rows<T, 4, NTH>(lds, rp_lds, nrows, kb, 128, hl, hn, sink); break;
        default: reduce_rows<T, 8, NTH>(lds, rp_lds, nrows, kb, 0, hl, hn, sink); return;
    }
    lds_barrier();
    const int n = *hn;
    if (n > 0) reduce_heavy_rows<T, NTH>(lds, rp_lds, kb, hl, n, sink);
}

template <typename T>
__device__ __forceinline__ T reduce_long(const T *lds, int a, int e, T *wsum) {
    const int tid = threadIdx.x;
    T s = T(0);
    for (int k = a + tid; k < e; k += kSpmvThreads) s += lds[k];
#pragma unroll
    for (int off = 32; off >= 1; off >>= 1) s = s + __shfl_xor(s, off, 64);
    if ((tid & 63) == 0) wsum[tid >> 6] = s;
    lds_barrier();
    return (wsum[0] + wsum[1]) + (wsum[2] + wsum[3]);
}

#ifdef RSP_SPMV_PROBE_LOADS
#include "spmv_probe.h"
#endif

#if defined(__HIP_DEVICE_COMPILE__) && !defined(__gfx950__) && !defined(__gfx942__)
#error "longrow_arrive's relaxed hand-off is only valid on gfx942 / gfx950"
#endif
template <typename T>
__device__ __forceinline__ void longrow_arrive(const SpmvBlock blk, const int *__restrict__ rowptr,
                                               T *partials, T *__restrict__ y, T t, T alpha, T beta,
                                               bool beta_nz) {
    typedef typename std::conditional<sizeof(T) == 8, unsigned long long, unsigned int>::type U;
    constexpr int C = SpmvTile<T>::kChunk;
    const int lane = threadIdx.x & 63;
    const int slot = -(blk.r1 + 1);
    const int rs = rowptr[blk.r0], re = rowptr[blk.r0 + 1];
    const int first = slot - (blk.k0 - rs) / C;
    const int n = (re - rs + C - 1) / C;
    typedef __attribute__((address_space(1))) U GU;
    typedef __attribute__((address_space(1))) unsigned int GI;
    GU *pv = (GU *)reinterpret_cast<U *>(partials);
    GI *ticket = (GI *)reinterpret_cast<unsigned int *>(partials + 2 * first + 1);
    unsigned int arrived = 0;
    if (lane == 0) {
        __hip_atomic_store(pv + 2 * slot, __builtin_bit_cast(U, t), __ATOMIC_RELAXED, __HIP_MEMORY_SCOPE_AGENT);
        asm volatile("s_waitcnt vmcnt(0)" ::: "memory");
        arrived = __hip_atomic_fetch_add(ticket, 1u, __ATOMIC_RELAXED, __HIP_MEMORY_SCOPE_AGENT);
    }
    arrived = (unsigned int)__builtin_amdgcn_readfirstlane((int)arrived);
    if (arrived != (unsigned int)(n - 1)) return;
    T s = T(0);
    for (int c0 = 0; c0 < n; c0 += 64) {
        const T p = c0 + lane < n ? __builtin_bit_cast(T, __hip_atomic_load(pv + 2 * (first + c0 + lane),
                                                                            __ATOMIC_RELAXED, __HIP_MEMORY_SCOPE_AGENT))
                                  : T(0);
        const int cn = min(64, n - c0);
        for (int c = 0; c < cn; ++c) s += __shfl(p, c, 64);
    }
    if (lane == 0) {
        T out = alpha * s;
        if (beta_nz) out += beta * y[blk.r0];
        y[blk.r0] = out;
        __hip_atomic_store(ticket, 0u, __ATOMIC_RELAXED, __HIP_MEMORY_SCOPE_AGENT);
    }
}

template <typename T, bool NT, bool BETA>
__device__ __forceinline__ void spmv_tile(
    const SpmvBlock blk, const int *__restrict__ rowptr, const int *__restrict__ colidx,
    const unsigned short *__restrict__ cidx, const int *__restrict__ runs, int cbase, int poff, int cmax,
    const T *__restrict__ vals, const T *__restrict__ x, T *__restrict__ y,
    T *partials, T alpha, T beta, int beta_nonzero, int nnz, int vector_ok, T *lds,
    T *wsum, unsigned short *rp_lds, int *hl, int fuse) {
    constexpr int VW = 16 / sizeof(T);
    constexpr int RPQ = (SpmvTile<T>::kMaxRows + kSpmvThreads) / kSpmvThreads;
    constexpr int RPW = (SpmvTile<T>::kMaxRows / 2 + kSpmvThreads) / kSpmvThreads;
    static_assert(RPW <= RPQ, "the packed row words fit the row offsets' registers");
    const int tid = threadIdx.x;
    const int k0 = blk.k0, k1 = blk.k1;
    const bool staged = cbase <= -2;
    constexpr int SMAX = SpmvTile<T>::kStageSlots / kSpmvThreads;
    int2 rd = make_int2(0, 0);
    int nr = 0;
    int lsl[SMAX];
    if (staged) {
        const int code = -2 - cbase;
        nr = code & 255;
        if (SpmvTile<T>::kStageList && nr == 255) {
            rd = reinterpret_cast<const int2 *>(runs)[code >> 8];
            const unsigned short *lst = reinterpret_cast<const unsigned short *>(runs + 2 * (code >> 8) + 2);
#pragma unroll
            for (int k = 0; k < SMAX; ++k)
                if (k * kSpmvThreads < rd.y) lsl[k] = lst[min(k * kSpmvThreads + tid, rd.y - 1)];
        } else if (tid <= nr) {
            rd = reinterpret_cast<const int2 *>(runs)[(code >> 8) + tid];
        }
    }
    const int nrows = blk.r1 - blk.r0;
    const int nrows_ld = nrows > 0 ? nrows : 0;
    const bool vec = vector_ok && k1 > k0 && k1 <= (nnz & ~(VW - 1));
    const int kb = vec ? (k0 & ~(VW - 1)) : k0;
    const unsigned int *rec =
        vec && staged && poff >= 0 ? reinterpret_cast<const unsigned int *>(runs) + (poff >> 1) : nullptr;
    const bool prow = rec && (poff & 1);
    const int nrw = (nrows_ld + 2) >> 1;
    const int *rsrc = prow ? reinterpret_cast<const int *>(rec) +
                                 kSpmvThreads * rsp_pack::words_per_thread(SpmvTile<T>::kSlots / kSpmvThreads)
                           : rowptr + blk.r0;
    const int rlim = prow ? nrw - 1 : nrows_ld;
    int rpv[RPQ];
#pragma unroll
    for (int q = 0; q < RPQ; ++q)
        rpv[q] = rsrc[min(tid + q * kSpmvThreads, rlim)];
#ifdef RSP_SPMV_PROBE_LOADS
    if (vec) {
        probe_tile_loads<T, NT>(colidx, vals, y, blk, kb, k1, rpv[0]);
        return;
    }
#endif
    if (vec && cbase >= 0)
        stream_products<T, NT, true>(colidx, cidx, cbase, cmax, vals, x, kb, k1, lds);
    else if (vec && staged && sizeof(T) == 4)
        stream_products_staged<T, NT, 2>(cidx, rec, rd, nr, lsl, vals, x, kb, k1, lds);
    else if (vec && rec)
        stream_products_staged<T, NT, 1>(cidx, rec, rd, nr, lsl, vals, x, kb, k1, lds);
    else if (vec && staged)
        stream_products_staged<T, NT, 0>(cidx, rec, rd, nr, lsl, vals, x, kb, k1, lds);
    else if (vec)
        stream_products<T, NT>(colidx, cidx, 0, 0, vals, x, kb, k1, lds);
    else
        stream_products_scalar<T>(colidx, vals, x, k0, kb, k1, lds);
    if (prow) {
#pragma unroll
        for (int q = 0; q < RPW; ++q) {
            const int i = tid + q * kSpmvThreads;
            if (i < nrw) reinterpret_cast<unsigned int *>(rp_lds)[i] = (unsigned int)rpv[q];
        }
    } else {
#pragma unroll
        for (int q = 0; q < RPQ; ++q) {
            const int i = tid + q * kSpmvThreads;
            if (i <= nrows) rp_lds[i] = (unsigned short)(rpv[q] - kb);
        }
    }
    if (tid == 0) hl[0] = 0;
    lds_barrier();

    if (blk.r1 < 0) {
        const T t = reduce_long(lds, k0 - kb, k1 - kb, wsum);
        if (blk.r1 != rsp::kSpmvWholeRow && fuse) {
            if (tid < 64) longrow_arrive<T>(blk, rowptr, partials, y, t, alpha, beta, BETA);
        } else if (tid == 0) {
            if (blk.r1 == rsp::kSpmvWholeRow) {
                T out = alpha * t;
                if (BETA) out += beta * y[blk.r0];
                y[blk.r0] = out;
            } else {
                partials[2 * -(blk.r1 + 1)] = t;
            }
        }
        return;
    }

    const int r0 = blk.r0;
    reduce_tile_rows<T>(lds, rp_lds, nrows, k1 - k0, 0, hl + 1, hl, [&](int rr, T sum) {
        T out = alpha * sum;
        if (BETA) out += beta * y[r0 + rr];
        constexpr bool kNtY = RSP_NT_Y > 0 || (RSP_NT_Y < 0 && sizeof(T) == 8);
        if constexpr (kNtY)
            __builtin_nontemporal_store(out, y + r0 + rr);
        else
            y[r0 + rr] = out;
    });
}

template <typename T, bool NT, bool BETA>
__global__ __launch_bounds__(kSpmvThreads) void spmv_tiles(
    const int *__restrict__ rowptr, const int *__restrict__ colidx, const T *__restrict__ vals,
    const T *__restrict__ x, T *__restrict__ y, const SpmvBlock *__restrict__ blocks, int nblocks,
    const int *__restrict__ cbases, const int *__restrict__ poffs, const unsigned short *__restrict__ cidx,
    const int *__restrict__ runs, int cmax, T *partials, T alpha, T beta, int beta_nonzero, int nnz,
    int vector_ok, int fuse) {
    __shared__ __attribute__((aligned(16))) T lds[SpmvTile<T>::kSlots];
    __shared__ T wsum[kSpmvThreads / 64];
    __shared__ int hl[1 + kSpmvHeavyMax];
    __shared__ __attribute__((aligned(4))) unsigned short rp_lds[SpmvTile<T>::kMaxRows + 2];
    const int b = xcd_swizzle(blockIdx.x, nblocks);
    spmv_tile<T, NT, BETA>(blocks[b], rowptr, colidx, cidx, runs, cbases[b], poffs[b], cmax, vals, x, y,
                           partials, alpha, beta, beta_nonzero, nnz, vector_ok, lds, wsum, rp_lds, hl,
                           fuse);
}

template <typename T>
__device__ __forceinline__ void fixup_row(const SpmvLongRow r, const T *__restrict__ partials,
                                          T *__restrict__ y, T alpha, T beta, int beta_nonzero) {
    const int lane = threadIdx.x;
    const T yv = (beta_nonzero && lane == 0) ? y[r.row] : T(0);
    T s = T(0);
    for (int c0 = 0; c0 < r.nchunks; c0 += 64) {
        const T p = c0 + lane < r.nchunks ? partials[2 * (r.first + c0 + lane)] : T(0);
        const int cn = min(64, r.nchunks - c0);
        for (int c = 0; c < cn; ++c) s += __shfl(p, c, 64);
    }
    if (lane == 0) {
        T out = alpha * s;
        if (beta_nonzero) out += beta * yv;
        y[r.row] = out;
    }
}

template <typename T>
__global__ __launch_bounds__(64) void spmv_longrow_fixup(const SpmvLongRow *__restrict__ lr,
                                                          int nlong, const T *__restrict__ partials,
                                                          T *__restrict__ y, T alpha, T beta,
                                                          int beta_nonzero) {
    fixup_row<T>(lr[blockIdx.x], partials, y, alpha, beta, beta_nonzero);
}

template <typename T, bool NT, bool BETA, bool SWZ>
__global__ __launch_bounds__(kSpmvThreads) void spmv_tiles_batch(
    const SpmvBatchEntry *__restrict__ entries, const SpmvBlock *__restrict__ tiles,
    const int *__restrict__ cbases, const int *__restrict__ poffs, SpmvBatchTable at, T alpha, T beta,
    int fuse) {
    __shared__ __attribute__((aligned(16))) T lds[SpmvTile<T>::kSlots];
    __shared__ T wsum[kSpmvThreads / 64];
    __shared__ int hl[1 + kSpmvHeavyMax];
    __shared__ __attribute__((aligned(4))) unsigned short rp_lds[SpmvTile<T>::kMaxRows + 2];
    const int b = blockIdx.x;
    int j = 0, lo = 0, hi = at.begin[1];
#pragma unroll
    for (int q = 1; q < kSpmvBatchMax; ++q)
        if (b >= at.begin[q]) {
            j = q;
            lo = at.begin[q];
            hi = at.begin[q + 1];
        }
    const int t = lo + (SWZ ? xcd_swizzle(b - lo, hi - lo) : b - lo);
    const SpmvBatchEntry e = entries[j];
    spmv_tile<T, NT, BETA>(tiles[t], e.rowptr, e.colidx, e.cidx, e.runs, cbases[t], poffs[t], e.cmax,
                           (const T *)e.vals, (const T *)e.x,
                           (T *)e.y, (T *)e.partials, alpha, beta, BETA, e.nnz, e.vector_ok, lds,
                           wsum, rp_lds, hl, fuse);
}

template <typename T>
__global__ __launch_bounds__(64) void spmv_longrow_fixup_batch(
    const SpmvBatchEntry *__restrict__ entries, const SpmvLongRow *__restrict__ lr,
    SpmvBatchTable at, T alpha, T beta, int beta_nonzero) {
    const int i = blockIdx.x;
    int j = 0;
#pragma unroll
    for (int q = 1; q < kSpmvBatchMax; ++q)
        if (i >= at.begin[q]) j = q;
    const SpmvBatchEntry e = entries[j];
    fixup_row<T>(lr[i], (const T *)e.partials, (T *)e.y, alpha, beta, beta_nonzero);
}

template <typename T>
static hipError_t launch_spmv_batch(const SpmvBatchArgs &a, hipStream_t s) {
    const T alpha = (T)a.alpha, beta = (T)a.beta;
    const int bnz = a.beta != 0.0;
    const int ntiles = a.tiles_at.begin[a.count];
    const int fuse = !(a.variant & rsp::kSpmvVariantFixup);
    if (ntiles > 0) {
        const bool nt = !(a.variant & 1), swz = !(a.variant & 8);
        auto kern = bnz ? (nt ? (swz ? spmv_tiles_batch<T, true, true, true>
                                     : spmv_tiles_batch<T, true, true, false>)
                              : (swz ? spmv_tiles_batch<T, false, true, true>
                                     : spmv_tiles_batch<T, false, true, false>))
                        : (nt ? (swz ? spmv_tiles_batch<T, true, false, true>
                                     : spmv_tiles_batch<T, true, false, false>)
                              : (swz ? spmv_tiles_batch<T, false, false, true>
                                     : spmv_tiles_batch<T, false, false, false>));
        hipLaunchKernelGGL(kern, dim3(ntiles), dim3(kSpmvThreads), 0, s, a.entries, a.tiles,
                           a.cbases, a.poffs, a.tiles_at, alpha, beta, fuse);
        const hipError_t e = hipGetLastError();
        if (e != hipSuccess) return e;
    }
    const int nlong = a.longs_at.begin[a.count];
    if (nlong > 0 && !fuse) {
        SpmvBatchTable lt = a.longs_at;
        lt.begin[kSpmvBatchMax] = nlong;
        hipLaunchKernelGGL((spmv_longrow_fixup_batch<T>), dim3(nlong), dim3(64), 0, s,
                           a.entries, a.longrows, lt, alpha, beta, bnz);
        return hipGetLastError();
    }
    return hipSuccess;
}

hipError_t spmv_batch_f32(const SpmvBatchArgs &a, hipStream_t s) {
    return launch_spmv_batch<float>(a, s);
}

template <typename T>
static hipError_t launch_spmv(const SpmvArgs &a, hipStream_t s) {
    if (a.nblocks <= 0) return hipSuccess;
    const T alpha = (T)a.alpha, beta = (T)a.beta;
    const int bnz = a.beta != 0.0;
    const int fuse = !(a.variant & rsp::kSpmvVariantFixup);
    auto kern = (a.variant & 1) ? (bnz ? spmv_tiles<T, false, true> : spmv_tiles<T, false, false>)
                                : (bnz ? spmv_tiles<T, true, true> : spmv_tiles<T, true, false>);
    hipLaunchKernelGGL(kern, dim3(a.nblocks), dim3(kSpmvThreads), 0, s, a.rowptr, a.colidx,
                       (const T *)a.vals, (const T *)a.x, (T *)a.y, a.blocks, a.nblocks, a.cbases,
                       a.poffs, a.cidx, a.runs, a.cmax, (T *)a.partials, alpha, beta, bnz, a.nnz, a.vector_ok, fuse);
    hipError_t e = hipGetLastError();
    if (e != hipSuccess) return e;
    if (a.nlong > 0 && !fuse) {
        hipLaunchKernelGGL((spmv_longrow_fixup<T>), dim3(a.nlong), dim3(64), 0, s,
                           a.longrows, a.nlong, (const T *)a.partials, (T *)a.y, alpha, beta, bnz);
        e = hipGetLastError();
    }
    return e;
}

hipError_t spmv_f32(const SpmvArgs &a, hipStream_t s) { return launch_spmv<float>(a, s); }
void warm_spmv() {
    hipFuncAttributes at;
    (void)hipFuncGetAttributes(&at, reinterpret_cast<const void *>(spmv_tiles<float, true, false>));
    int o = 0;
    (void)hipOccupancyMaxActiveBlocksPerMultiprocessor(&o, spmv_tiles<float, true, false>, kSpmvThreads, 0);
}

#ifndef RSP_FTZ_BUILD
int spmv_tiles_per_cu(int elem_bytes) {
    int o = 0;
    const hipError_t e =
        elem_bytes == 8
            ? hipOccupancyMaxActiveBlocksPerMultiprocessor(&o, spmv_tiles<double, true, false>, kSpmvThreads, 0)
            : hipOccupancyMaxActiveBlocksPerMultiprocessor(&o, spmv_tiles<float, true, false>, kSpmvThreads, 0);
    return (e == hipSuccess && o > 0) ? o : 1;
}

template <typename E>
__global__ __launch_bounds__(256) void gather_kernel(const int64_t *__restrict__ idx,
                                                     const E *__restrict__ src, E *__restrict__ dst,
                                                     int64_t n) {
    const int64_t stride = (int64_t)gridDim.x * 256;
    for (int64_t i = (int64_t)blockIdx.x * 256 + threadIdx.x; i < n; i += stride) dst[i] = src[idx[i]];
}

template <typename E>
__global__ __launch_bounds__(256) void scatter_kernel(const int64_t *__restrict__ idx,
                                                      const E *__restrict__ src, E *__restrict__ dst,
                                                      int64_t n) {
    const int64_t stride = (int64_t)gridDim.x * 256;
    for (int64_t i = (int64_t)blockIdx.x * 256 + threadIdx.x; i < n; i += stride) dst[idx[i]] = src[i];
}

hipError_t scatter(int elem_bytes, int64_t n, const int64_t *idx, const void *src, void *dst,
                   hipStream_t s) {
    if (n <= 0) return hipSuccess;
    const int64_t want = (n + 255) / 256;
    const int grid = (int)(want < 2048 ? want : 2048);
    if (elem_bytes == 8)
        hipLaunchKernelGGL((scatter_kernel<double>), dim3(grid), dim3(256), 0, s, idx,
                           (const double *)src, (double *)dst, n);
    else
        hipLaunchKernelGGL((scatter_kernel<float>), dim3(grid), dim3(256), 0, s, idx,
                           (const float *)src, (float *)dst, n);
    return hipGetLastError();
}

hipError_t gather(int elem_bytes, int64_t n, const int64_t *idx, const void *src, void *dst,
                  hipStream_t s) {
    if (n <= 0) return hipSuccess;
    const int64_t want = (n + 255) / 256;
    const int grid = (int)(want < 2048 ? want : 2048);
    if (elem_bytes == 8)
        hipLaunchKernelGGL((gather_kernel<double>), dim3(grid), dim3(256), 0, s, idx,
                           (const double *)src, (double *)dst, n);
    else
        hipLaunchKernelGGL((gather_kernel<float>), dim3(grid), dim3(256), 0, s, idx,
                           (const float *)src, (float *)dst, n);
    return hipGetLastError();
}

hipError_t spmv_f64(const SpmvArgs &a, hipStream_t s) { return launch_spmv<double>(a, s); }
hipError_t spmv_batch_f64(const SpmvBatchArgs &a, hipStream_t s) {
    return launch_spmv_batch<double>(a, s);
}
#endif

}
```

### respasol_amd/csrc/spmv_probe.h

```cpp
#pragma once

template <typename T, bool NT>
__device__ __forceinline__ void probe_tile_loads(const int *__restrict__ colidx, const T *__restrict__ vals,
                                                 T *__restrict__ y, const SpmvBlock blk, int kb, int k1, int rp0) {
    constexpr int VW = 16 / sizeof(T);
    typedef typename VecT<T, VW>::V V;
    typedef typename VecT<T, VW>::I I;
    constexpr int IT = SpmvTile<T>::kSlots / (kSpmvThreads * VW);
    const int tid = threadIdx.x;
    const int last = (k1 - 1) & ~(VW - 1);
    T acc = T(0);
#pragma unroll
    for (int it = 0; it < IT; ++it) {
        const int e = min(kb + (it * kSpmvThreads + tid) * VW, last);
        const I c = ld<NT>(reinterpret_cast<const I *>(colidx + e));
        const V v = ld<NT>(reinterpret_cast<const V *>(vals + e));
#pragma unroll
        for (int j = 0; j < VW; ++j) acc += v[j] + T(c[j]);
    }
    if (acc == T(-12345.0)) y[blk.r0] = acc + T(rp0);
}
```

Measured before the change: 1031 GFLOP/s.

## Pack tile metadata into single record and add optional lookahead prefetch

Merges the per-tile block bounds, cbase and poff arrays into one 24-byte SpmvRec record so each workgroup reads its tile descriptor from one place instead of three separate arrays. It also adds an env-controlled lookahead (default 0) that lets a workgroup touch a later tile's metadata, plus host-side validation of the block-to-tile index mapping. Record reads lose 16-byte alignment, and the validation adds host work at plan time.

```diff
diff --git a/respasol_amd/csrc/rsp_api.cpp b/respasol_amd/csrc/rsp_api.cpp
--- a/respasol_amd/csrc/rsp_api.cpp
+++ b/respasol_amd/csrc/rsp_api.cpp
@@ -1,5 +1,6 @@
 
 #include "rsp_internal.h"
+#include "spmv_lookahead.h"
 #include "spmv_pack.h"
 
 #include <atomic>
@@ -8,6 +9,7 @@
 
 using rsp::SpmvBlock;
 using rsp::SpmvLongRow;
+using rsp::SpmvRec;
 using rsp::SpmvTile;
 
 namespace {
@@ -32,15 +34,13 @@
 }
 
 struct SpmvLayout {
-    size_t off_long, off_part, off_cbase, off_poff, off_cidx, off_runs, bytes;
+    size_t off_long, off_part, off_cidx, off_runs, bytes;
 };
 static SpmvLayout spmv_layout(const SpmvBounds &b, size_t elem, int64_t nnz, size_t run_ints = 0) {
     SpmvLayout l;
-    l.off_long = align256(b.nblocks * sizeof(SpmvBlock));
+    l.off_long = align256(b.nblocks * sizeof(SpmvRec));
     l.off_part = l.off_long + align256(b.nlong * sizeof(SpmvLongRow));
-    l.off_cbase = l.off_part + align256(b.nslots * 2 * elem);
-    l.off_poff = l.off_cbase + align256(b.nblocks * sizeof(int));
-    l.off_cidx = l.off_poff + align256(b.nblocks * sizeof(int));
+    l.off_cidx = l.off_part + align256(b.nslots * 2 * elem);
     l.off_runs = l.off_cidx + align256((size_t)std::max<int64_t>(nnz, 0) * sizeof(uint16_t));
     l.bytes = l.off_runs + align256(run_ints * sizeof(int));
     return l;
@@ -328,6 +328,55 @@
     }
 }
 
+static void tile_records(const TilePlan &p, int t0, int t1, SpmvRec *out) {
+    for (int t = t0; t < t1; t++) {
+        const SpmvBlock &b = p.blocks[(size_t)t];
+        out[t - t0] = SpmvRec{b.r0, b.r1, b.k0, b.k1, p.cbase[(size_t)t], p.poff[(size_t)t]};
+    }
+}
+
+static int spmv_lookahead_env() {
+    return rsp_la::clamp_lookahead(env_int("RSP_SPMV_LOOKAHEAD", rsp::kSpmvLookahead));
+}
+
+static bool launch_indices_ok(const rsp::SpmvBatchTable &at, int count, int ntiles, int D) {
+    if (count < 0 || count > rsp::kSpmvBatchMax || ntiles < 0) return false;
+    if (count > 0 && (at.begin[0] != 0 || at.begin[count] != ntiles)) return false;
+    for (int q = 0; q < count; q++)
+        if (at.begin[q] < 0 || at.begin[q] > at.begin[q + 1]) return false;
+    for (int q = count + 1; q <= rsp::kSpmvBatchMax; q++)
+        if (at.begin[q] != INT_MAX) return false;
+    if (count == 0) return ntiles == 0;
+    std::vector<char> seen((size_t)ntiles);
+    for (int swz = 0; swz < 2; swz++) {
+        std::fill(seen.begin(), seen.end(), 0);
+        for (int b = 0; b < ntiles; b++) {
+            int j = -1, lo = 0, hi = 0;
+            const int t = rsp_la::tile_of<rsp::kSpmvBatchMax>(at.begin, b, swz != 0, &j, &lo, &hi);
+            if (j < 0 || j >= count || lo != at.begin[j] || hi != at.begin[j + 1] || t < lo || t >= hi ||
+                seen[(size_t)t])
+                return false;
+            seen[(size_t)t] = 1;
+            for (int d : {D, 1}) {
+                const int bt = rsp_la::target_block(b, d, ntiles);
+                if (bt == -1) continue;
+                if (bt <= b || bt >= ntiles) return false;
+                const int tt = rsp_la::tile_ahead<rsp::kSpmvBatchMax>(at.begin, bt, swz != 0, j, lo, hi);
+                if (tt < 0 || tt >= ntiles) return false;
+            }
+        }
+    }
+    return true;
+}
+
+static bool launch_indices_ok(int n, int D) {
+    rsp::SpmvBatchTable at;
+    for (int q = 0; q <= rsp::kSpmvBatchMax; q++) at.begin[q] = INT_MAX;
+    at.begin[0] = 0;
+    at.begin[1] = n;
+    return launch_indices_ok(at, 1, n, D);
+}
+
 static rsp_status_t download_pattern(rsp_handle_t h, rsp_spmat_t mat, rsp_an::hvec<int> &rp,
                                      rsp_an::hvec<int> &ci) {
     const int m = (int)mat->rows;
@@ -373,8 +422,11 @@
     const rsp_an::hvec<SpmvBlock> &blocks = p.blocks;
     const rsp_an::hvec<SpmvLongRow> &longrows = p.longrows;
     const int nslots = p.nslots, nint = p.nint;
-    const rsp_an::hvec<int> &cbase = p.cbase;
     const rsp_an::hvec<uint16_t> &c16 = p.c16;
+    for (int n : {(int)blocks.size(), nint, (int)blocks.size() - nint})
+        if (!launch_indices_ok(n, h->spmv_lookahead)) return RSP_STATUS_INTERNAL_ERROR;
+    rsp_an::hvec<SpmvRec> recs(blocks.size());
+    tile_records(p, 0, (int)blocks.size(), recs.data());
     const int64_t nnz_c16 = p.nnz_c16;
     SpmvBounds b{blocks.size(), longrows.size(), (size_t)nslots};
     const SpmvLayout lay = spmv_layout(b, elem_size(compute_type), (int64_t)c16.size(), p.runs.size());
@@ -395,11 +447,7 @@
     }
     char *buf = (char *)mat->d_plan;
     if (!blocks.empty()) {
-        RSP_CHECK_HIP(hipMemcpyAsync(buf, blocks.data(), blocks.size() * sizeof(SpmvBlock),
-                                     hipMemcpyHostToDevice, h->stream));
-        RSP_CHECK_HIP(hipMemcpyAsync(buf + lay.off_cbase, cbase.data(), cbase.size() * sizeof(int),
-                                     hipMemcpyHostToDevice, h->stream));
-        RSP_CHECK_HIP(hipMemcpyAsync(buf + lay.off_poff, p.poff.data(), p.poff.size() * sizeof(int),
+        RSP_CHECK_HIP(hipMemcpyAsync(buf, recs.data(), recs.size() * sizeof(SpmvRec),
                                      hipMemcpyHostToDevice, h->stream));
     }
     if (!c16.empty())
@@ -427,10 +475,9 @@
     mat->nnz_s = m > 0 ? rp[(size_t)m] : 0;
     mat->off_long = off_long;
     mat->off_part = off_part;
-    mat->off_cbase = lay.off_cbase;
-    mat->off_poff = lay.off_poff;
     mat->off_cidx = lay.off_cidx;
     mat->off_runs = lay.off_runs;
+    mat->la_checked = h->spmv_lookahead;
     mat->nnz_c16 = nnz_c16;
     mat->nnz_staged = p.nnz_staged;
     return RSP_STATUS_SUCCESS;
@@ -449,6 +496,11 @@
         rsp_status_t st = spmv_plan(h, mat, compute_type);
         if (st != RSP_STATUS_SUCCESS) return st;
     }
+    if (mat->la_checked != h->spmv_lookahead) {
+        for (int n : {mat->nblocks, mat->nint, mat->nblocks - mat->nint})
+            if (!launch_indices_ok(n, h->spmv_lookahead)) return RSP_STATUS_INTERNAL_ERROR;
+        mat->la_checked = h->spmv_lookahead;
+    }
     char *plan = (char *)mat->d_plan;
     rsp::SpmvArgs a;
     a.m = (int)mat->rows;
@@ -457,10 +509,8 @@
     a.vals = mat->vals;
     a.x = d_x;
     a.y = d_y;
-    a.blocks = (const SpmvBlock *)plan;
+    a.blocks = (const SpmvRec *)plan;
     a.nblocks = mat->nblocks;
-    a.cbases = (const int *)(plan + mat->off_cbase);
-    a.poffs = (const int *)(plan + mat->off_poff);
     a.cidx = (const unsigned short *)(plan + mat->off_cidx);
     a.runs = (const int *)(plan + mat->off_runs);
     a.cmax = mat->cols > 0 ? (int)(mat->cols - 1) : 0;
@@ -481,14 +531,13 @@
             a.nlong = 0;
         } else {
             a.blocks += mat->nint;
-            a.cbases += mat->nint;
-            a.poffs += mat->nint;
             a.nblocks = mat->nblocks - mat->nint;
         }
     }
     a.vector_ok = ((((uintptr_t)mat->colidx) | ((uintptr_t)mat->vals)) & 15) == 0;
     a.nnz = mat->nnz_s;
     a.variant = h->spmv_variant;
+    a.lookahead = h->spmv_lookahead;
     hipError_t e;
     if (compute_type == RSP_R_64F)
         e = rsp_k::spmv_f64(a, h->stream);
@@ -506,6 +555,7 @@
     rsp_an::hvec<rsp::SpmvBatchArgs> launches;
     void *d_mem = nullptr;
     int64_t tiles = 0, entries_16bit = 0;
+    rsp_an::hvec<int> la_checked;
     ~rsp_spmv_batch() {
         if (d_mem) (void)hipFree(d_mem);
     }
@@ -539,7 +589,7 @@
     const bool spread_ok = !(h->spmv_variant & 16), c16_ok = !(h->spmv_variant & 32);
     const bool stage_ok = !(h->spmv_variant & rsp::kSpmvVariantNoStage);
     rsp_an::hvec<TilePlan> plans((size_t)count);
-    struct Span { int first, count; size_t off_e, off_t, off_c, off_k, off_l; rsp_an::hvec<size_t> off_16, off_p, off_r; };
+    struct Span { int first, count; size_t off_e, off_t, off_l; rsp_an::hvec<size_t> off_16, off_p, off_r; };
     rsp_an::hvec<Span> spans;
     size_t bytes = 0;
     auto tile_range = [part](const TilePlan &p, int *t0, int *t1) {
@@ -547,7 +597,7 @@
         *t1 = part == 1 ? p.nint : (int)p.blocks.size();
     };
     for (int first = 0; first < count; first += rsp::kSpmvBatchMax) {
-        Span sp{first, std::min(rsp::kSpmvBatchMax, count - first), 0, 0, 0, 0, 0, {}, {}, {}};
+        Span sp{first, std::min(rsp::kSpmvBatchMax, count - first), 0, 0, 0, {}, {}, {}};
         rsp_an::hvec<rsp_an::hvec<int>> rps((size_t)sp.count), cis((size_t)sp.count);
         int64_t nt_full = 0, nnz_all = 0;
         for (int q = 0; q < sp.count; q++) {
@@ -584,11 +634,7 @@
         sp.off_e = bytes;
         bytes += (size_t)sp.count * sizeof(rsp::SpmvBatchEntry);
         sp.off_t = bytes;
-        bytes += (size_t)nt * sizeof(SpmvBlock);
-        sp.off_c = bytes;
-        bytes += ((size_t)nt * sizeof(int) + 15) & ~(size_t)15;
-        sp.off_k = bytes;
-        bytes += ((size_t)nt * sizeof(int) + 15) & ~(size_t)15;
+        bytes += ((size_t)nt * sizeof(SpmvRec) + 15) & ~(size_t)15;
         sp.off_l = bytes;
         bytes += ((size_t)nl * sizeof(SpmvLongRow) + 15) & ~(size_t)15;
         for (int q = 0; q < sp.count; q++) {
@@ -622,8 +668,8 @@
                 nl += part == 1 ? 0 : (int)plans[sp.first + q].longrows.size();
             }
             bool ok = region(sp.off_e, (size_t)sp.count * sizeof(rsp::SpmvBatchEntry)) &&
-                      region(sp.off_t, (size_t)nt * sizeof(SpmvBlock)) && region(sp.off_c, (size_t)nt * sizeof(int)) &&
-                      region(sp.off_k, (size_t)nt * sizeof(int)) && region(sp.off_l, (size_t)nl * sizeof(SpmvLongRow));
+                      region(sp.off_t, (size_t)nt * sizeof(SpmvRec)) &&
+                      region(sp.off_l, (size_t)nl * sizeof(SpmvLongRow));
             for (int q = 0; ok && q < sp.count; q++) ok = region(sp.off_16[q], plans[sp.first + q].c16.size() * 2);
             for (int q = 0; ok && q < sp.count; q++) ok = region(sp.off_r[q], plans[sp.first + q].runs.size() * 4);
             for (int q = 0; ok && q < sp.count; q++)
@@ -636,9 +682,7 @@
     for (const Span &sp : spans) {
         rsp::SpmvBatchArgs a{};
         a.entries = (const rsp::SpmvBatchEntry *)((char *)b->d_mem + sp.off_e);
-        a.tiles = (const SpmvBlock *)((char *)b->d_mem + sp.off_t);
-        a.cbases = (const int *)((char *)b->d_mem + sp.off_c);
-        a.poffs = (const int *)((char *)b->d_mem + sp.off_k);
+        a.tiles = (const SpmvRec *)((char *)b->d_mem + sp.off_t);
         a.longrows = (const SpmvLongRow *)((char *)b->d_mem + sp.off_l);
         a.count = sp.count;
         for (int q = 0; q <= rsp::kSpmvBatchMax; q++)
@@ -668,14 +712,8 @@
             for (int t = t0; t < t1; t++)
                 if (p.cbase[(size_t)t] != -1) b->entries_16bit += p.blocks[(size_t)t].k1 - p.blocks[(size_t)t].k0;
             b->tiles += t1 - t0;
-            if (t1 > t0) {
-                memcpy(host.data() + sp.off_t + (size_t)nt * sizeof(SpmvBlock), p.blocks.data() + t0,
-                       (size_t)(t1 - t0) * sizeof(SpmvBlock));
-                memcpy(host.data() + sp.off_c + (size_t)nt * sizeof(int), p.cbase.data() + t0,
-                       (size_t)(t1 - t0) * sizeof(int));
-                memcpy(host.data() + sp.off_k + (size_t)nt * sizeof(int), p.poff.data() + t0,
-                       (size_t)(t1 - t0) * sizeof(int));
-            }
+            if (t1 > t0)
+                tile_records(p, t0, t1, reinterpret_cast<SpmvRec *>(host.data() + sp.off_t) + nt);
             if (nlq > 0)
                 memcpy(host.data() + sp.off_l + (size_t)nl * sizeof(SpmvLongRow), p.longrows.data(),
                        (size_t)nlq * sizeof(SpmvLongRow));
@@ -688,6 +726,7 @@
         }
         a.tiles_at.begin[sp.count] = nt;
         a.longs_at.begin[sp.count] = nl;
+        if (!launch_indices_ok(a.tiles_at, sp.count, nt, h->spmv_lookahead)) return RSP_STATUS_INTERNAL_ERROR;
         b->launches.push_back(a);
     }
     if (bytes > 0) {
@@ -698,6 +737,7 @@
         b->mats.push_back(mats[j]);
         b->plan_gen.push_back(mats[j]->plan_gen);
     }
+    b->la_checked.push_back(h->spmv_lookahead);
     *batch = b.release();
     return RSP_STATUS_SUCCESS;
 }
@@ -752,11 +792,14 @@
     int vw, iw;
     pack_geometry(type, &vw, &iw);
     const int pack_mode = spmv_pack_mode();
-    if (p.poff.size() != p.blocks.size()) return RSP_STATUS_INTERNAL_ERROR;
+    if (p.poff.size() != p.blocks.size() || p.cbase.size() != p.blocks.size()) return RSP_STATUS_INTERNAL_ERROR;
+    if (!launch_indices_ok((int)p.blocks.size(), spmv_lookahead_env())) return RSP_STATUS_INTERNAL_ERROR;
+    rsp_an::hvec<SpmvRec> recs(p.blocks.size());
+    tile_records(p, 0, (int)p.blocks.size(), recs.data());
     int64_t npk = 0, epk = 0;
-    for (size_t t = 0; t < p.blocks.size(); t++) {
-        const SpmvBlock &b = p.blocks[t];
-        const int cb = p.cbase[t], po = p.poff[t];
+    for (size_t t = 0; t < recs.size(); t++) {
+        const SpmvRec &b = recs[t];
+        const int cb = b.cbase, po = b.poff;
         const uint32_t *rec = nullptr;
         if (po >= 0) {
             const int nrows = b.r1 - b.r0, kb = b.k0 & ~(vw - 1);
@@ -864,6 +907,7 @@
     c->ftz = 0;
     const char *v = getenv("RSP_SPMV_VARIANT");
     c->spmv_variant = v ? atoi(v) : 0;
+    c->spmv_lookahead = spmv_lookahead_env();
     c->num_cus = prop.multiProcessorCount > 0 ? prop.multiProcessorCount : 256;
     rsp_k::warm_spmv();
     rsp_k_ftz::warm_spmv();
@@ -1061,10 +1105,17 @@
     const double av = b->type == RSP_R_64F ? *(const double *)alpha : *(const float *)alpha;
     const double bv = b->type == RSP_R_64F ? *(const double *)beta : *(const float *)beta;
     if (b->part != 0 && bv != 0.0) return RSP_STATUS_INVALID_VALUE;
+    if (std::find(b->la_checked.begin(), b->la_checked.end(), h->spmv_lookahead) == b->la_checked.end()) {
+        for (const rsp::SpmvBatchArgs &a : b->launches)
+            if (!launch_indices_ok(a.tiles_at, a.count, a.tiles_at.begin[a.count], h->spmv_lookahead))
+                return RSP_STATUS_INTERNAL_ERROR;
+        b->la_checked.push_back(h->spmv_lookahead);
+    }
     for (rsp::SpmvBatchArgs a : b->launches) {
         a.alpha = av;
         a.beta = bv;
         a.variant = h->spmv_variant;
+        a.lookahead = h->spmv_lookahead;
         hipError_t e;
         if (b->type == RSP_R_64F)
             e = rsp_k::spmv_batch_f64(a, h->stream);
diff --git a/respasol_amd/csrc/rsp_internal.h b/respasol_amd/csrc/rsp_internal.h
--- a/respasol_amd/csrc/rsp_internal.h
+++ b/respasol_amd/csrc/rsp_internal.h
@@ -23,6 +23,7 @@
     hipStream_t stream;
     int ftz;
     int spmv_variant;
+    int spmv_lookahead;
     int num_cus;
     unsigned long long *d_ftrace;
     unsigned long long *d_strace;
@@ -46,11 +47,12 @@
     int nblocks, nlong, nslots;
     int nnz_s;
     size_t off_long, off_part;
-    size_t off_cbase, off_poff, off_cidx, off_runs;
+    size_t off_cidx, off_runs;
     int64_t nnz_c16;
     int64_t nnz_staged;
     int64_t local_cols;
     int nint;
+    int la_checked;
     unsigned long long plan_gen;
 };
 
diff --git a/respasol_amd/csrc/rsp_kernels.h b/respasol_amd/csrc/rsp_kernels.h
--- a/respasol_amd/csrc/rsp_kernels.h
+++ b/respasol_amd/csrc/rsp_kernels.h
@@ -8,6 +8,11 @@
 struct alignas(16) SpmvBlock {
     int r0, r1, k0, k1;
 };
+
+struct alignas(8) SpmvRec {
+    int r0, r1, k0, k1, cbase, poff;
+};
+static_assert(sizeof(SpmvRec) == 24, "rsp_spmv_plan_stats counts 24 B per tile");
 
 struct alignas(16) SpmvLongRow {
     int row, first, nchunks, pad;
@@ -50,12 +55,10 @@
     const void *vals;
     const void *x;
     void *y;
-    const SpmvBlock *blocks;
+    const SpmvRec *blocks;
     int nblocks;
-    const int *cbases;
     const unsigned short *cidx;
     const int *runs;
-    const int *poffs;
     int cmax;
     const SpmvLongRow *longrows;
     int nlong;
@@ -63,6 +66,7 @@
     double alpha, beta;
     int nnz;
     int vector_ok;
+    int lookahead;
     int variant;
 };
 
@@ -85,17 +89,17 @@
 };
 struct SpmvBatchArgs {
     const SpmvBatchEntry *entries;
-    const SpmvBlock *tiles;
-    const int *cbases;
-    const int *poffs;
+    const SpmvRec *tiles;
     const SpmvLongRow *longrows;
     int count;
     SpmvBatchTable tiles_at, longs_at;
     double alpha, beta;
+    int lookahead;
     int variant;
 };
 constexpr int kSpmvVariantFixup = 256;
 constexpr int kSpmvVariantNoStage = 1024;
+constexpr int kSpmvLookahead = 0;
 
 struct LevelSeg {
     int lb, le, thin, c0, c1;
diff --git a/respasol_amd/csrc/spmv.hip b/respasol_amd/csrc/spmv.hip
--- a/respasol_amd/csrc/spmv.hip
+++ b/respasol_amd/csrc/spmv.hip
@@ -4,6 +4,7 @@
 #include <type_traits>
 
 #include "rsp_kernels.h"
+#include "spmv_lookahead.h"
 #include "spmv_pack.h"
 
 #ifndef RSP_KNS
@@ -20,6 +21,8 @@
 using rsp::kSpmvHeavyMax;
 using rsp::SpmvArgs;
 using rsp::SpmvBlock;
+using rsp::SpmvRec;
+using rsp_la::xcd_swizzle;
 using rsp::SpmvLongRow;
 using rsp::SpmvTile;
 using rsp::kSpmvBatchMax;
@@ -42,12 +45,13 @@
     typedef unsigned short __attribute__((ext_vector_type(4))) H;
 };
 
-__device__ __forceinline__ int xcd_swizzle(int bid, int nwg) {
-    const int q = nwg >> 3, r = nwg & 7;
-    const int xcd = bid & 7, idx = bid >> 3;
-    const int start = xcd < r ? xcd * (q + 1) : r * (q + 1) + (xcd - r) * q;
-    return start + idx;
-}
+
+__device__ __forceinline__ int touch_word(const int *p) {
+    int w = 0;
+    if (p) asm volatile("s_load_dword %0, %1, 0x0" : "=s"(w) : "s"(p));
+    return w;
+}
+__device__ __forceinline__ void touch_end(int w) { asm volatile("s_waitcnt lgkmcnt(0)" ::"s"(w)); }
 
 template <bool NT, typename P>
 __device__ __forceinline__ P ld(const P *p) {
@@ -63,7 +67,7 @@
                                                 const unsigned short *__restrict__ cidx, int cbase,
                                                 int cmax, const T *__restrict__ vals,
                                                 const T *__restrict__ x, int kb, int k1,
-                                                T *__restrict__ lds) {
+                                                T *__restrict__ lds, const int *__restrict__ touch, int &tw) {
     constexpr int VW = 16 / sizeof(T);
     typedef typename VecT<T, VW>::V V;
     typedef typename VecT<T, VW>::I I;
@@ -86,6 +90,7 @@
         const int e = min(kb + (it * NTH + tid) * VW, last);
         vv[it] = ld<NT>(reinterpret_cast<const V *>(vals + e));
     }
+    tw = touch_word(touch);
     __builtin_amdgcn_sched_barrier(0);
     T xv[IT][VW];
 #pragma unroll
@@ -122,7 +127,8 @@
                                                        int nr, const int (&lsl)[SpmvTile<T>::kStageSlots / NTH],
                                                        const T *__restrict__ vals,
                                                        const T *__restrict__ x, int kb, int k1,
-                                                       T *__restrict__ lds) {
+                                                       T *__restrict__ lds, const int *__restrict__ touch,
+                                                       int &tw) {
     constexpr int VW = 16 / sizeof(T);
     constexpr int SMAX = SpmvTile<T>::kStageSlots / NTH;
     typedef typename VecT<T, VW>::V V;
@@ -193,6 +199,7 @@
                 xs[k] = xload(r.x + (us[k] - r.y));
             }
     }
+    tw = touch_word(touch);
 #pragma unroll
     for (int k = 0; k < SMAX; ++k)
         if (k * NTH < U && k * NTH + tid < U) lds[k * NTH + tid] = xs[k];
@@ -322,7 +329,7 @@
     return (wsum[0] + wsum[1]) + (wsum[2] + wsum[3]);
 }
 
-#ifdef RSP_SPMV_PROBE_LOADS
+#if defined(RSP_SPMV_PROBE_LOADS) || defined(RSP_SPMV_PROBE_TRIP)
 #include "spmv_probe.h"
 #endif
 
@@ -370,7 +377,7 @@
 
 template <typename T, bool NT, bool BETA>
 __device__ __forceinline__ void spmv_tile(
-    const SpmvBlock blk, const int *__restrict__ rowptr, const int *__restrict__ colidx,
+    const SpmvBlock blk, const int *__restrict__ touch, const int *__restrict__ rowptr, const int *__restrict__ colidx,
     const unsigned short *__restrict__ cidx, const int *__restrict__ runs, int cbase, int poff, int cmax,
     const T *__restrict__ vals, const T *__restrict__ x, T *__restrict__ y,
     T *partials, T alpha, T beta, int beta_nonzero, int nnz, int vector_ok, T *lds,
@@ -421,18 +428,21 @@
         return;
     }
 #endif
+    int tw = 0;
     if (vec && cbase >= 0)
-        stream_products<T, NT, true>(colidx, cidx, cbase, cmax, vals, x, kb, k1, lds);
+        stream_products<T, NT, true>(colidx, cidx, cbase, cmax, vals, x, kb, k1, lds, touch, tw);
     else if (vec && staged && sizeof(T) == 4)
-        stream_products_staged<T, NT, 2>(cidx, rec, rd, nr, lsl, vals, x, kb, k1, lds);
+        stream_products_staged<T, NT, 2>(cidx, rec, rd, nr, lsl, vals, x, kb, k1, lds, touch, tw);
     else if (vec && rec)
-        stream_products_staged<T, NT, 1>(cidx, rec, rd, nr, lsl, vals, x, kb, k1, lds);
+        stream_products_staged<T, NT, 1>(cidx, rec, rd, nr, lsl, vals, x, kb, k1, lds, touch, tw);
     else if (vec && staged)
-        stream_products_staged<T, NT, 0>(cidx, rec, rd, nr, lsl, vals, x, kb, k1, lds);
+        stream_products_staged<T, NT, 0>(cidx, rec, rd, nr, lsl, vals, x, kb, k1, lds, touch, tw);
     else if (vec)
-        stream_products<T, NT>(colidx, cidx, 0, 0, vals, x, kb, k1, lds);
-    else
+        stream_products<T, NT>(colidx, cidx, 0, 0, vals, x, kb, k1, lds, touch, tw);
+    else {
         stream_products_scalar<T>(colidx, vals, x, k0, kb, k1, lds);
+        tw = touch_word(touch);
+    }
     if (prow) {
 #pragma unroll
         for (int q = 0; q < RPW; ++q) {
@@ -448,6 +458,7 @@
     }
     if (tid == 0) hl[0] = 0;
     lds_barrier();
+    touch_end(tw);
 
     if (blk.r1 < 0) {
         const T t = reduce_long(lds, k0 - kb, k1 - kb, wsum);
@@ -480,18 +491,20 @@
 template <typename T, bool NT, bool BETA>
 __global__ __launch_bounds__(kSpmvThreads) void spmv_tiles(
     const int *__restrict__ rowptr, const int *__restrict__ colidx, const T *__restrict__ vals,
-    const T *__restrict__ x, T *__restrict__ y, const SpmvBlock *__restrict__ blocks, int nblocks,
-    const int *__restrict__ cbases, const int *__restrict__ poffs, const unsigned short *__restrict__ cidx,
-    const int *__restrict__ runs, int cmax, T *partials, T alpha, T beta, int beta_nonzero, int nnz,
-    int vector_ok, int fuse) {
+    const T *__restrict__ x, T *__restrict__ y, const SpmvRec *__restrict__ blocks, int nblocks,
+    const unsigned short *__restrict__ cidx, const int *__restrict__ runs, int cmax, T *partials, T alpha,
+    T beta, int beta_nonzero, int nnz, int vector_ok, int fuse, int la) {
     __shared__ __attribute__((aligned(16))) T lds[SpmvTile<T>::kSlots];
     __shared__ T wsum[kSpmvThreads / 64];
     __shared__ int hl[1 + kSpmvHeavyMax];
     __shared__ __attribute__((aligned(4))) unsigned short rp_lds[SpmvTile<T>::kMaxRows + 2];
     const int b = xcd_swizzle(blockIdx.x, nblocks);
-    spmv_tile<T, NT, BETA>(blocks[b], rowptr, colidx, cidx, runs, cbases[b], poffs[b], cmax, vals, x, y,
-                           partials, alpha, beta, beta_nonzero, nnz, vector_ok, lds, wsum, rp_lds, hl,
-                           fuse);
+    const SpmvRec rec = blocks[b];
+    const int bt = rsp_la::target_block(blockIdx.x, la, nblocks);
+    const int *touch = bt >= 0 ? &blocks[xcd_swizzle(bt, nblocks)].r0 : nullptr;
+    spmv_tile<T, NT, BETA>(SpmvBlock{rec.r0, rec.r1, rec.k0, rec.k1}, touch, rowptr, colidx, cidx,
+                           runs, rec.cbase, rec.poff, cmax, vals, x, y, partials, alpha, beta, beta_nonzero,
+                           nnz, vector_ok, lds, wsum, rp_lds, hl, fuse);
 }
 
 template <typename T>
@@ -522,26 +535,36 @@
 
 template <typename T, bool NT, bool BETA, bool SWZ>
 __global__ __launch_bounds__(kSpmvThreads) void spmv_tiles_batch(
-    const SpmvBatchEntry *__restrict__ entries, const SpmvBlock *__restrict__ tiles,
-    const int *__restrict__ cbases, const int *__restrict__ poffs, SpmvBatchTable at, T alpha, T beta,
-    int fuse) {
+    const SpmvBatchEntry *__restrict__ entries, const SpmvRec *__restrict__ tiles, SpmvBatchTable at,
+    T alpha, T beta, int fuse, int la, int ngrid
+#ifdef RSP_SPMV_PROBE_TRIP
+    , const int *__restrict__ trip
+#endif
+) {
     __shared__ __attribute__((aligned(16))) T lds[SpmvTile<T>::kSlots];
     __shared__ T wsum[kSpmvThreads / 64];
     __shared__ int hl[1 + kSpmvHeavyMax];
     __shared__ __attribute__((aligned(4))) unsigned short rp_lds[SpmvTile<T>::kMaxRows + 2];
     const int b = blockIdx.x;
-    int j = 0, lo = 0, hi = at.begin[1];
-#pragma unroll
-    for (int q = 1; q < kSpmvBatchMax; ++q)
-        if (b >= at.begin[q]) {
-            j = q;
-            lo = at.begin[q];
-            hi = at.begin[q + 1];
-        }
-    const int t = lo + (SWZ ? xcd_swizzle(b - lo, hi - lo) : b - lo);
+    int j, lo, hi;
+    const int t = rsp_la::tile_of<kSpmvBatchMax>(at.begin, b, SWZ, &j, &lo, &hi);
     const SpmvBatchEntry e = entries[j];
-    spmv_tile<T, NT, BETA>(tiles[t], e.rowptr, e.colidx, e.cidx, e.runs, cbases[t], poffs[t], e.cmax,
-                           (const T *)e.vals, (const T *)e.x,
+#ifdef RSP_SPMV_PROBE_TRIP
+    const SpmvRec rec = tiles[t + (trip ? probe_trip_word(trip, t) : 0)];
+#else
+    const SpmvRec rec = tiles[t];
+#endif
+    const int bt = rsp_la::target_block(b, la, ngrid);
+    const int *touch = nullptr;
+    if (bt >= 0) {
+        const int tt = rsp_la::tile_ahead<kSpmvBatchMax>(at.begin, bt, SWZ, j, lo, hi);
+        touch = &tiles[tt].r0;
+#ifdef RSP_SPMV_PROBE_TRIP
+        if (trip) touch = trip + (size_t)tt * 32;
+#endif
+    }
+    spmv_tile<T, NT, BETA>(SpmvBlock{rec.r0, rec.r1, rec.k0, rec.k1}, touch, e.rowptr, e.colidx,
+                           e.cidx, e.runs, rec.cbase, rec.poff, e.cmax, (const T *)e.vals, (const T *)e.x,
                            (T *)e.y, (T *)e.partials, alpha, beta, BETA, e.nnz, e.vector_ok, lds,
                            wsum, rp_lds, hl, fuse);
 }
@@ -575,8 +598,16 @@
                                      : spmv_tiles_batch<T, true, false, false>)
                               : (swz ? spmv_tiles_batch<T, false, false, true>
                                      : spmv_tiles_batch<T, false, false, false>));
-        hipLaunchKernelGGL(kern, dim3(ntiles), dim3(kSpmvThreads), 0, s, a.entries, a.tiles,
-                           a.cbases, a.poffs, a.tiles_at, alpha, beta, fuse);
+        const int la = rsp_la::clamp_lookahead(a.lookahead);
+#ifdef RSP_SPMV_PROBE_TRIP
+        const int *trip = (a.variant & 2048) ? probe_trip_scratch(ntiles, s) : nullptr;
+        if ((a.variant & 2048) && !trip) return hipErrorOutOfMemory;
+        hipLaunchKernelGGL(kern, dim3(ntiles), dim3(kSpmvThreads), 0, s, a.entries, a.tiles, a.tiles_at,
+                           alpha, beta, fuse, la, ntiles, trip);
+#else
+        hipLaunchKernelGGL(kern, dim3(ntiles), dim3(kSpmvThreads), 0, s, a.entries, a.tiles, a.tiles_at,
+                           alpha, beta, fuse, la, ntiles);
+#endif
         const hipError_t e = hipGetLastError();
         if (e != hipSuccess) return e;
     }
@@ -604,8 +635,9 @@
     auto kern = (a.variant & 1) ? (bnz ? spmv_tiles<T, false, true> : spmv_tiles<T, false, false>)
                                 : (bnz ? spmv_tiles<T, true, true> : spmv_tiles<T, true, false>);
     hipLaunchKernelGGL(kern, dim3(a.nblocks), dim3(kSpmvThreads), 0, s, a.rowptr, a.colidx,
-                       (const T *)a.vals, (const T *)a.x, (T *)a.y, a.blocks, a.nblocks, a.cbases,
-                       a.poffs, a.cidx, a.runs, a.cmax, (T *)a.partials, alpha, beta, bnz, a.nnz, a.vector_ok, fuse);
+                       (const T *)a.vals, (const T *)a.x, (T *)a.y, a.blocks, a.nblocks, a.cidx, a.runs,
+                       a.cmax, (T *)a.partials, alpha, beta, bnz, a.nnz, a.vector_ok, fuse,
+                       rsp_la::clamp_lookahead(a.lookahead));
     hipError_t e = hipGetLastError();
     if (e != hipSuccess) return e;
     if (a.nlong > 0 && !fuse) {
diff --git a/respasol_amd/csrc/spmv_lookahead.h b/respasol_amd/csrc/spmv_lookahead.h
--- /dev/null
+++ b/respasol_amd/csrc/spmv_lookahead.h
@@ -0,0 +1,55 @@
+#pragma once
+
+#if defined(__HIPCC__)
+#define RSP_LA_HD __host__ __device__ __forceinline__
+#else
+#define RSP_LA_HD inline
+#endif
+
+namespace rsp_la {
+
+constexpr int kXcds = 8;
+constexpr int kMaxLookahead = 1 << 16;
+
+RSP_LA_HD int xcd_swizzle(int bid, int nwg) {
+    const int q = nwg >> 3, r = nwg & 7;
+    const int xcd = bid & 7, idx = bid >> 3;
+    const int start = xcd < r ? xcd * (q + 1) : r * (q + 1) + (xcd - r) * q;
+    return start + idx;
+}
+
+template <int N>
+RSP_LA_HD int tile_of(const int (&begin)[N + 1], int b, bool swz, int *jm, int *lom, int *him) {
+    int j = 0, lo = 0, hi = begin[1];
+#if defined(__HIPCC__)
+#pragma unroll
+#endif
+    for (int q = 1; q < N; ++q)
+        if (b >= begin[q]) {
+            j = q;
+            lo = begin[q];
+            hi = begin[q + 1];
+        }
+    *jm = j;
+    *lom = lo;
+    *him = hi;
+    return lo + (swz ? xcd_swizzle(b - lo, hi - lo) : b - lo);
+}
+
+template <int N>
+RSP_LA_HD int tile_ahead(const int *begin, int bt, bool swz, int j, int lo, int hi) {
+    for (; bt >= hi && j + 1 < N; ++j) {
+        lo = hi;
+        hi = begin[j + 2];
+    }
+    return lo + (swz ? xcd_swizzle(bt - lo, hi - lo) : bt - lo);
+}
+
+RSP_LA_HD int clamp_lookahead(int D) { return D < 0 ? 0 : D > kMaxLookahead ? kMaxLookahead : D; }
+
+RSP_LA_HD int target_block(int b, int D, int grid) {
+    if (D <= 0 || D > kMaxLookahead) return -1;
+    return b < grid - kXcds * D ? b + kXcds * D : -1;
+}
+
+}
diff --git a/respasol_amd/csrc/spmv_probe.h b/respasol_amd/csrc/spmv_probe.h
--- a/respasol_amd/csrc/spmv_probe.h
+++ b/respasol_amd/csrc/spmv_probe.h
@@ -1,5 +1,25 @@
 #pragma once
 
+#ifdef RSP_SPMV_PROBE_TRIP
+__device__ __forceinline__ int probe_trip_word(const int *__restrict__ trip, int t) {
+    return trip[(size_t)t * 32];
+}
+static const int *probe_trip_scratch(int ntiles, hipStream_t s) {
+    static int *buf = nullptr;
+    static int cap = 0;
+    if (ntiles > cap) {
+        if (buf) (void)hipFree(buf);
+        buf = nullptr;
+        cap = 0;
+        if (hipMalloc(&buf, (size_t)ntiles * 128) != hipSuccess) return nullptr;
+        if (hipMemsetAsync(buf, 0, (size_t)ntiles * 128, s) != hipSuccess) return nullptr;
+        cap = ntiles;
+    }
+    return buf;
+}
+#endif
+
+#ifdef RSP_SPMV_PROBE_LOADS
 template <typename T, bool NT>
 __device__ __forceinline__ void probe_tile_loads(const int *__restrict__ colidx, const T *__restrict__ vals,
                                                  T *__restrict__ y, const SpmvBlock blk, int kb, int k1, int rp0) {
@@ -20,3 +40,4 @@
     }
     if (acc == T(-12345.0)) y[blk.r0] = acc + T(rp0);
 }
+#endif
diff --git a/respasol_amd/drivers/spmv_lookahead_check.cpp b/respasol_amd/drivers/spmv_lookahead_check.cpp
--- /dev/null
+++ b/respasol_amd/drivers/spmv_lookahead_check.cpp
@@ -0,0 +1,138 @@
+#include <limits.h>
+#include <stdio.h>
+
+#include <vector>
+
+#include "spmv_lookahead.h"
+
+namespace {
+
+constexpr int kMax = 32;
+
+struct Table {
+    int begin[kMax + 1];
+};
+
+Table make_table(const std::vector<int> &sizes) {
+    Table t;
+    for (int q = 0; q <= kMax; q++) t.begin[q] = INT_MAX;
+    int at = 0;
+    for (size_t q = 0; q < sizes.size(); q++) {
+        t.begin[q] = at;
+        at += sizes[q];
+    }
+    t.begin[sizes.size()] = at;
+    return t;
+}
+
+std::vector<int> simulate_tiles(const std::vector<int> &sizes, bool swz) {
+    std::vector<int> tile;
+    int lo = 0;
+    for (int n : sizes) {
+        std::vector<int> next(8), t((size_t)n);
+        int at = lo;
+        for (int x = 0; x < 8; x++) {
+            next[(size_t)x] = at;
+            at += n / 8 + (x < n % 8);
+        }
+        for (int i = 0; i < n; i++) t[(size_t)i] = swz ? next[(size_t)(i & 7)]++ : lo + i;
+        tile.insert(tile.end(), t.begin(), t.end());
+        lo += n;
+    }
+    return tile;
+}
+
+int simulate_target(int b, int D, int grid) {
+    if (D <= 0) return -1;
+    int at = b;
+    for (int step = 0; step < D; step++) {
+        at += 8;
+        if (at >= grid) return -1;
+    }
+    return at;
+}
+
+int check_launch(const std::vector<int> &sizes, int D, bool swz) {
+    const Table tb = make_table(sizes);
+    const std::vector<int> want = simulate_tiles(sizes, swz);
+    const int grid = (int)want.size();
+    std::vector<int> rec((size_t)grid);
+    for (int t = 0; t < grid; t++) rec[(size_t)t] = t;
+    std::vector<char> seen((size_t)grid, 0);
+    for (int b = 0; b < grid; b++) {
+        int j = -1, lo = -1, hi = -1;
+        const int t = rsp_la::tile_of<kMax>(tb.begin, b, swz, &j, &lo, &hi);
+        if (t != want[(size_t)b] || j < 0 || j >= (int)sizes.size() || lo != tb.begin[j] || hi != tb.begin[j + 1] ||
+            t < lo || t >= hi) {
+            printf("FAIL: %zu matrices, swz %d: block %d -> tile %d of matrix %d, want %d\n", sizes.size(), (int)swz,
+                   b, t, j, want[(size_t)b]);
+            return 1;
+        }
+        if (rec[(size_t)t] != t || seen[(size_t)t]++) {
+            printf("FAIL: %zu matrices, swz %d: tile %d taken twice\n", sizes.size(), (int)swz, t);
+            return 1;
+        }
+        const int bt = rsp_la::target_block(b, D, grid), wt = simulate_target(b, D, grid);
+        if (bt != wt) {
+            printf("FAIL: %zu matrices, D %d: block %d looks ahead at %d, want %d\n", sizes.size(), D, b, bt, wt);
+            return 1;
+        }
+        if (bt >= 0) {
+            const int tt = rsp_la::tile_ahead<kMax>(tb.begin, bt, swz, j, lo, hi);
+            int j2, lo2, hi2;
+            if (tt != want[(size_t)bt] || rec[(size_t)tt] != tt ||
+                tt != rsp_la::tile_of<kMax>(tb.begin, bt, swz, &j2, &lo2, &hi2)) {
+                printf("FAIL: %zu matrices, D %d: target block %d -> tile %d, want %d\n", sizes.size(), D, bt, tt,
+                       want[(size_t)bt]);
+                return 1;
+            }
+        }
+    }
+    if (sizes.size() == 1 && swz)
+        for (int b = 0; b < grid; b++)
+            if (rsp_la::xcd_swizzle(b, grid) != want[(size_t)b]) {
+                printf("FAIL: xcd_swizzle(%d, %d)\n", b, grid);
+                return 1;
+            }
+    return 0;
+}
+
+}
+
+int main() {
+    const int edge[] = {0, 1, 7, 8, 9};
+    std::vector<std::vector<int>> launches;
+    for (int n : edge) launches.push_back({n});
+    for (int n : {15, 16, 17, 64, 300, 2049}) launches.push_back({n});
+    for (int a : edge)
+        for (int b : edge) launches.push_back({a, b});
+    launches.push_back({300, 0});
+    launches.push_back({0, 300});
+    for (int count : {15, 32}) {
+        std::vector<int> cyc, big, empty_ends;
+        for (int q = 0; q < count; q++) {
+            cyc.push_back(edge[q % 5]);
+            big.push_back(q % 3 == 0 ? 0 : 37 * q + edge[q % 5]);
+            empty_ends.push_back(q == 0 || q == count - 1 ? 0 : 9 + q);
+        }
+        launches.push_back(cyc);
+        launches.push_back(big);
+        launches.push_back(empty_ends);
+        launches.push_back(std::vector<int>((size_t)count, 0));
+        launches.push_back(std::vector<int>((size_t)count, 1));
+    }
+    int bad = 0, n = 0;
+    for (const std::vector<int> &sizes : launches)
+        for (int D : {0, 1, 3, 256})
+            for (bool swz : {true, false}) {
+                bad += check_launch(sizes, D, swz);
+                n++;
+            }
+    for (int D : {-1, INT_MAX, rsp_la::kMaxLookahead + 1})
+        for (int b : {0, 1, 99})
+            bad += rsp_la::target_block(b, D, 100) != -1;
+    bad += rsp_la::target_block(0, 1, INT_MAX) != 8 || rsp_la::target_block(INT_MAX - 8, 1, INT_MAX) != -1 ||
+           rsp_la::target_block(INT_MAX - 9, 1, INT_MAX) != INT_MAX - 1;
+    printf("%s: %d launches\n", bad ? "FAILED" : "ok", n);
+    return bad ? 1 : 0;
+}
```

After: 1030 GFLOP/s. About the same (-0.2%).
